# SymbioticLab/Oobleck

Measured on AMD Instinct MI355X. Metric: tokens/sec (whole node) GPT-2 1F1B, higher is better.
Workload: dtype bf16; 1 GPU; gpt2.yaml GPT-2-small 1F1B, global microbatch 128x1024 tokens, bf16; model=gpt2, global_batch=128, seq_len=1024, parallelism=pp1dp1

## Files before the change

include/oobleck_stage.h:

```cpp
#ifndef OOBLECK_STAGE_H
#define OOBLECK_STAGE_H

#include <stdint.h>

#ifdef __cplusplus
extern "C" {
#endif

enum {
  OB_KIND_EMBED = 0,
  OB_KIND_BLOCK = 1,
  OB_KIND_FINAL = 2
};

typedef struct ob_layer* ob_layer_t;

typedef struct {
  int32_t kind;
  int32_t n_embd;
  int32_t n_head;
  int32_t n_positions;
  int32_t vocab_size;
  int32_t max_batch;
  int32_t seq_len;
  int32_t n_slots;
  int32_t dtype;
} ob_layer_desc;

int64_t ob_layer_param_count(const ob_layer_desc* desc);

int ob_layer_create(const ob_layer_desc* desc, ob_layer_t* out);

enum {
  OB_DROP_EMBD = 0,
  OB_DROP_ATTN = 1,
  OB_DROP_RESID_ATTN = 2,
  OB_DROP_RESID_MLP = 3
};

typedef struct {
  float embd_pdrop;
  float resid_pdrop;
  float attn_pdrop;
  int32_t layer_id;
  uint64_t seed;
} ob_dropout_desc;

int ob_layer_create_ex(const ob_layer_desc* desc, const ob_dropout_desc* drop,
                       ob_layer_t* out);

int ob_layer_uses_flash(ob_layer_t l);

int ob_layer_set_training(ob_layer_t l, int on);

int ob_layer_set_dropout_tick(ob_layer_t l, uint64_t tick);

int ob_layer_bind(ob_layer_t l, void* params, void* grads);

int ob_layer_set_batch(ob_layer_t l, int32_t batch);

int ob_layer_forward(ob_layer_t l, int32_t slot, const void* in, void* out,
                     const int64_t* labels, void* stream);

int ob_layer_backward(ob_layer_t l, int32_t slot, const void* dout, void* din,
                      void* stream);

int ob_layer_destroy(ob_layer_t l);

int ob_layer_refresh_weights(ob_layer_t l, void* stream);

int ob_adamw_step(void* p, const void* g, void* m, void* v, int64_t n,
                  int32_t step, float lr, float beta1, float beta2, float eps,
                  float weight_decay, void* stream);


int64_t ob_sqnorm_ws_count(const int64_t* counts, int32_t n);

int ob_sqnorm_multi_f32(const void* const* ptrs, const int64_t* counts,
                        const int32_t* out_index, int32_t n, void* ws,
                        void* out, void* stream);

int ob_clip_finish(const void* sq, int32_t n, float max_norm, void* stats,
                   void* stream);

int ob_adamw_step_scaled(void* p, const void* g, void* m, void* v, int64_t n,
                         int32_t step, float lr, float beta1, float beta2,
                         float eps, float weight_decay, const void* clip_stats,
                         void* stream);


int ob_gemm_f32(int transA, int transB, int64_t M, int64_t N, int64_t K,
                float alpha, const void* A, int64_t lda,
                int64_t strideA1, int64_t strideA2,
                const void* B, int64_t ldb,
                int64_t strideB1, int64_t strideB2,
                float beta, void* C, int64_t ldc,
                int64_t strideC1, int64_t strideC2,
                int64_t n1, int64_t n2,
                const void* bias, const void* residual, int atomic, int splitk,
                void* stream);

int ob_layernorm_fwd_f32(const void* x, const void* w, const void* b, void* y,
                         void* mean, void* rstd, int64_t rows, int64_t H,
                         float eps, void* stream);
int ob_layernorm_bwd_f32(const void* x, const void* w, const void* mean,
                         const void* rstd, const void* dy, void* dx,
                         void* dw, void* db, int64_t rows, int64_t H,
                         int dx_accum, void* stream);

int ob_softmax_causal_fwd_f32(void* scores, int64_t batch, int64_t S,
                              float scale, void* stream);
int ob_softmax_causal_bwd_f32(const void* P, void* dP, int64_t batch,
                              int64_t S, void* stream);

int ob_gelu_fwd_f32(const void* u, void* g, int64_t n, void* stream);
int ob_gelu_bwd_f32(const void* u, const void* dg, void* du, int64_t n,
                    void* stream);

int ob_colsum_f32(const void* X, void* db, int64_t M, int64_t N, void* stream);

int ob_dropout_mask(uint64_t seed, int32_t layer_id, int32_t site,
                    uint64_t tick, float p, int64_t n, void* keep_u8,
                    void* stream);
int ob_dropout_scale_f32(uint64_t seed, int32_t layer_id, int32_t site,
                         uint64_t tick, float p, const void* x, void* y,
                         int64_t n, void* stream);
int ob_dropout_scale_bf16(uint64_t seed, int32_t layer_id, int32_t site,
                          uint64_t tick, float p, const void* x, void* y,
                          int64_t n, void* stream);
int ob_dropout_add_f32(uint64_t seed, int32_t layer_id, int32_t site,
                       uint64_t tick, float p, const void* t, const void* res,
                       void* y, int64_t n, void* stream);
int ob_dropout_add_bf16(uint64_t seed, int32_t layer_id, int32_t site,
                        uint64_t tick, float p, const void* t,
                        const void* res, void* y, int64_t n, void* stream);
int ob_dropout_scale_colsum_f32(uint64_t seed, int32_t layer_id, int32_t site,
                                uint64_t tick, float p, const void* dy,
                                void* dm, void* db, int64_t M, int64_t N,
                                void* stream);
int ob_dropout_scale_colsum_bf16(uint64_t seed, int32_t layer_id, int32_t site,
                                 uint64_t tick, float p, const void* dy,
                                 void* dm, void* db, int64_t M, int64_t N,
                                 void* stream);

int ob_gemm_bf16(int transA, int transB, int64_t M, int64_t N, int64_t K,
                 float alpha, const void* A, int64_t lda,
                 int64_t strideA1, int64_t strideA2,
                 const void* B, int64_t ldb,
                 int64_t strideB1, int64_t strideB2,
                 float beta, void* C, int64_t ldc,
                 int64_t strideC1, int64_t strideC2,
                 int64_t n1, int64_t n2,
                 const void* bias, const void* residual, int out_kind,
                 int splitk, void* stream);
int ob_gemm_bf16_route(int transA, int transB, int64_t M, int64_t N, int64_t K,
                       int64_t n1, int64_t n2, int out_kind, int splitk,
                       float beta, int aligned16, int env_mask,
                       const char* force, int32_t* out);

int ob_flash_fwd_nt_bf16(const void* qkv, void* O, void* lse, int64_t B,
                         int64_t Sq, int64_t H, int64_t nh, float scale,
                         void* stream);
int ob_flash_bwd_nt_bf16(const void* qkv, const void* dO, const void* lse,
                         const void* D, void* dqkv, void* dbias_qkv,
                         int64_t B, int64_t Sq, int64_t H, int64_t nh,
                         float scale, void* stream);
int ob_flash_bwd_nt_d_bf16(const void* qkv, const void* O, const void* dO,
                           const void* lse, void* D_ws, void* dqkv,
                           void* dbias_qkv, int64_t B, int64_t Sq, int64_t H,
                           int64_t nh, float scale, void* stream);
int ob_flash_fwd_nt_drop_bf16(const void* qkv, void* O, void* lse, int64_t B,
                              int64_t Sq, int64_t H, int64_t nh, float scale,
                              uint64_t seed, int32_t layer_id, uint64_t tick,
                              float p, void* stream);
int ob_flash_bwd_nt_d_drop_bf16(const void* qkv, const void* O, const void* dO,
                                const void* lse, void* D_ws, void* dqkv,
                                void* dbias_qkv, int64_t B, int64_t Sq,
                                int64_t H, int64_t nh, float scale,
                                uint64_t seed, int32_t layer_id, uint64_t tick,
                                float p, void* stream);
int ob_flash_fold_rows(int64_t kind, int64_t Sq, int64_t block, int64_t unit,
                       int64_t* row0, int64_t* first_tile, int64_t* n_tiles);
int64_t ob_flash_fold_grid(int64_t kind, int64_t Sq, int64_t Z);
int ob_flash_fold_id(int64_t kind, int64_t Sq, int64_t Z, int64_t id,
                     int64_t* z, int64_t* block);

int ob_f32_to_bf16(const void* x, void* y, int64_t n, void* stream);
int ob_f32_to_bf16_t(const void* x, void* y, int64_t rows, int64_t cols,
                     void* stream);
int ob_bf16_to_f32(const void* x, void* y, int64_t n, void* stream);

void ob_profile_enable(int on);
void ob_profile_reset(void);
int ob_profile_read(int fam, double* total_ms, long long* count);

const char* ob_last_error(void);

const char* ob_build_arch(void);

#ifdef __cplusplus
}
#endif
#endif
```

oobleck_amd/_ext.py:

```python
from __future__ import annotations

import ctypes
import pathlib

_LIB = None
SO_PATH = pathlib.Path(__file__).resolve().parent / "libob_stage.so"


class ObLayerDesc(ctypes.Structure):
    _fields_ = [
        ("kind", ctypes.c_int32),
        ("n_embd", ctypes.c_int32),
        ("n_head", ctypes.c_int32),
        ("n_positions", ctypes.c_int32),
        ("vocab_size", ctypes.c_int32),
        ("max_batch", ctypes.c_int32),
        ("seq_len", ctypes.c_int32),
        ("n_slots", ctypes.c_int32),
        ("dtype", ctypes.c_int32),
    ]


class ObDropoutDesc(ctypes.Structure):
    _fields_ = [
        ("embd_pdrop", ctypes.c_float),
        ("resid_pdrop", ctypes.c_float),
        ("attn_pdrop", ctypes.c_float),
        ("layer_id", ctypes.c_int32),
        ("seed", ctypes.c_uint64),
    ]


DROP_EMBD, DROP_ATTN, DROP_RESID_ATTN, DROP_RESID_MLP = 0, 1, 2, 3


def _configure(lib: ctypes.CDLL) -> ctypes.CDLL:
    i64, i32, f32, vp = ctypes.c_int64, ctypes.c_int32, ctypes.c_float, ctypes.c_void_p
    lib.ob_last_error.restype = ctypes.c_char_p
    lib.ob_build_arch.restype = ctypes.c_char_p
    lib.ob_layer_param_count.restype = i64
    lib.ob_layer_param_count.argtypes = [ctypes.POINTER(ObLayerDesc)]
    lib.ob_layer_create.argtypes = [ctypes.POINTER(ObLayerDesc),
                                    ctypes.POINTER(vp)]
    u64 = ctypes.c_uint64
    lib.ob_layer_create_ex.argtypes = [ctypes.POINTER(ObLayerDesc),
                                       ctypes.POINTER(ObDropoutDesc),
                                       ctypes.POINTER(vp)]
    lib.ob_layer_set_training.argtypes = [vp, i32]
    lib.ob_layer_uses_flash.argtypes = [vp]
    lib.ob_layer_set_dropout_tick.argtypes = [vp, u64]
    key = [u64, i32, i32, u64, f32]
    lib.ob_dropout_mask.argtypes = key + [i64, vp, vp]
    lib.ob_dropout_scale_f32.argtypes = key + [vp, vp, i64, vp]
    lib.ob_dropout_scale_bf16.argtypes = key + [vp, vp, i64, vp]
    lib.ob_dropout_add_f32.argtypes = key + [vp, vp, vp, i64, vp]
    lib.ob_dropout_add_bf16.argtypes = key + [vp, vp, vp, i64, vp]
    lib.ob_dropout_scale_colsum_f32.argtypes = key + [vp, vp, vp, i64, i64, vp]
    lib.ob_dropout_scale_colsum_bf16.argtypes = key + [vp, vp, vp, i64, i64,
                                                       vp]
    lib.ob_layer_bind.argtypes = [vp, vp, vp]
    lib.ob_layer_set_batch.argtypes = [vp, i32]
    lib.ob_layer_forward.argtypes = [vp, i32, vp, vp, vp, vp]
    lib.ob_layer_backward.argtypes = [vp, i32, vp, vp, vp]
    lib.ob_layer_destroy.argtypes = [vp]
    lib.ob_layer_refresh_weights.argtypes = [vp, vp]
    lib.ob_adamw_step.argtypes = [vp, vp, vp, vp, i64, i32, f32, f32, f32,
                                  f32, f32, vp]
    lib.ob_sqnorm_ws_count.restype = i64
    lib.ob_sqnorm_ws_count.argtypes = [ctypes.POINTER(i64), i32]
    lib.ob_sqnorm_multi_f32.argtypes = [ctypes.POINTER(vp),
                                        ctypes.POINTER(i64),
                                        ctypes.POINTER(i32), i32, vp, vp, vp]
    lib.ob_clip_finish.argtypes = [vp, i32, f32, vp, vp]
    lib.ob_adamw_step_scaled.argtypes = [vp, vp, vp, vp, i64, i32, f32, f32,
                                         f32, f32, f32, vp, vp]
    lib.ob_gemm_f32.argtypes = [i32, i32, i64, i64, i64, f32, vp, i64, i64,
                                i64, vp, i64, i64, i64, f32, vp, i64, i64,
                                i64, i64, i64, vp, vp, i32, i32, vp]
    lib.ob_layernorm_fwd_f32.argtypes = [vp, vp, vp, vp, vp, vp, i64, i64,
                                         f32, vp]
    lib.ob_layernorm_bwd_f32.argtypes = [vp, vp, vp, vp, vp, vp, vp, vp, i64,
                                         i64, i32, vp]
    lib.ob_softmax_causal_fwd_f32.argtypes = [vp, i64, i64, f32, vp]
    lib.ob_softmax_causal_bwd_f32.argtypes = [vp, vp, i64, i64, vp]
    lib.ob_gelu_fwd_f32.argtypes = [vp, vp, i64, vp]
    lib.ob_gelu_bwd_f32.argtypes = [vp, vp, vp, i64, vp]
    lib.ob_colsum_f32.argtypes = [vp, vp, i64, i64, vp]
    lib.ob_gemm_bf16.argtypes = [i32, i32, i64, i64, i64, f32, vp, i64, i64,
                                 i64, vp, i64, i64, i64, f32, vp, i64, i64,
                                 i64, i64, i64, vp, vp, i32, i32, vp]
    lib.ob_f32_to_bf16.argtypes = [vp, vp, i64, vp]
    lib.ob_f32_to_bf16_t.argtypes = [vp, vp, i64, i64, vp]
    lib.ob_f32_to_bf16_t_ld.argtypes = [vp, vp, i64, i64, i64, vp]
    lib.ob_bf16_to_f32.argtypes = [vp, vp, i64, vp]
    lib.ob_gelu_fwd_bf16.argtypes = [vp, vp, i64, vp]
    lib.ob_gelu_bwd_bf16.argtypes = [vp, vp, vp, i64, vp]
    lib.ob_ce_fwd_bf16.argtypes = [vp, vp, vp, vp, i64, i64, i64, i64, vp]
    lib.ob_ce_bwd_bf16.argtypes = [vp, vp, vp, vp, i64, i64, i64, i64, vp]
    lib.ob_embed_fwd_bf16.argtypes = [vp, vp, vp, vp, i64, i64, i64, vp]
    lib.ob_embed_bwd_bf16.argtypes = [vp, vp, vp, vp, i64, i64, i64, vp]
    lib.ob_softmax_causal_fwd_bf16.argtypes = [vp, i64, i64, f32, vp]
    lib.ob_softmax_causal_bwd_bf16.argtypes = [vp, vp, i64, i64, vp]
    lib.ob_transpose_bf16.argtypes = [vp, vp, i64, i64, vp]
    lib.ob_gemm_lt_bias.argtypes = [i32, i32, i64, i64, i64, f32, vp, i64,
                                    vp, i64, f32, vp, i64, i32, vp, vp]
    lib.ob_gemm_lt_f32.argtypes = [i32, i32, i64, i64, i64, f32, vp, i64,
                                   vp, i64, f32, vp, i64, vp]
    lib.ob_flash_fwd_bf16.argtypes = [vp, vp, vp, vp, i64, i64, i64, i64,
                                      f32, vp]
    lib.ob_transpose_bf16_b.argtypes = [vp, vp, i64, i64, i64, i64, i64,
                                        i64, i64, vp]
    lib.ob_layernorm_fwd_bf16.argtypes = [vp, vp, vp, vp, vp, vp, i64, i64,
                                          f32, vp]
    lib.ob_layernorm_bwd_bf16.argtypes = [vp, vp, vp, vp, vp, vp, vp, vp,
                                          i64, i64, i32, vp]
    lib.ob_colsum_bf16.argtypes = [vp, vp, i64, i64, vp]
    lib.ob_layernorm_fwd_copy_bf16.argtypes = [vp, vp, vp, vp, vp, vp, vp,
                                               i64, i64, f32, vp]
    lib.ob_layernorm_bwd_res_bf16.argtypes = [vp, vp, vp, vp, vp, vp, vp, vp,
                                              vp, vp, vp, i64, i64, vp]
    lib.ob_gelu_bwd_colsum_bf16.argtypes = [vp, vp, vp, vp, i64, i64, vp]
    lib.ob_gemm_lt.argtypes = [i32, i32, i64, i64, i64, f32, vp, i64, vp,
                               i64, f32, vp, i64, i32, vp]
    lib.ob_gemm_bf16_nt_8ph.argtypes = [vp, vp, vp, vp, vp, i64, i64, i64,
                                        i64, i64, i64, i64, i64, i64, i64,
                                        i64, i64, i64, i64, f32, f32, i32,
                                        i32, vp, i64]
    lib.ob_gemm_bf16_route.argtypes = [i32, i32, i64, i64, i64, i64, i64, i32,
                                       i32, f32, i32, i32, ctypes.c_char_p,
                                       ctypes.POINTER(ctypes.c_int32)]
    lib.ob_profile_enable.argtypes = [i32]
    lib.ob_profile_enable.restype = None
    lib.ob_profile_reset.argtypes = []
    lib.ob_profile_reset.restype = None
    lib.ob_profile_read.argtypes = [i32, ctypes.POINTER(ctypes.c_double),
                                    ctypes.POINTER(ctypes.c_longlong)]
    lib.ob_flash_dsum_bf16.argtypes = [vp, vp, vp, i64, i64, i64, i64, vp]
    lib.ob_flash_bwd_bf16.argtypes = [vp, vp, vp, vp, vp, vp, vp, vp, i64,
                                      i64, i64, i64, f32, vp]
    lib.ob_flash_fwd_nt_bf16.argtypes = [vp, vp, vp, i64, i64, i64, i64,
                                         f32, vp]
    lib.ob_flash_bwd_nt_bf16.argtypes = [vp, vp, vp, vp, vp, vp, i64, i64,
                                         i64, i64, f32, vp]
    lib.ob_flash_bwd_nt_d_bf16.argtypes = [vp, vp, vp, vp, vp, vp, vp, i64,
                                           i64, i64, i64, f32, vp]
    lib.ob_flash_fwd_nt_drop_bf16.argtypes = [vp, vp, vp, i64, i64, i64, i64,
                                              f32, u64, i32, u64, f32, vp]
    lib.ob_flash_bwd_nt_d_drop_bf16.argtypes = [vp, vp, vp, vp, vp, vp, vp,
                                                i64, i64, i64, i64, f32, u64,
                                                i32, u64, f32, vp]
    p64 = ctypes.POINTER(ctypes.c_int64)
    lib.ob_flash_fold_rows.argtypes = [i64, i64, i64, i64, p64, p64, p64]
    lib.ob_flash_fold_grid.argtypes = [i64, i64, i64]
    lib.ob_flash_fold_grid.restype = ctypes.c_int64
    lib.ob_flash_fold_id.argtypes = [i64, i64, i64, i64, p64, p64]
    return lib


def get_ext(build_if_missing: bool = True) -> ctypes.CDLL:
    global _LIB
    if _LIB is not None:
        return _LIB
    if not SO_PATH.exists():
        if build_if_missing:
            from .build import build
            try:
                build()
            except Exception as e:
                raise RuntimeError(
                    f"oobleck_amd: HIP extension missing and build failed: {e}. "
                    "The hot path has no fallback — run __graft_entry__.build().") from e
        else:
            raise RuntimeError(
                "oobleck_amd: HIP extension libob_stage.so is missing. "
                "The hot path has no fallback — run __graft_entry__.build().")
    _LIB = _configure(ctypes.CDLL(str(SO_PATH)))
    return _LIB


def check(rc: int, what: str = "") -> None:
    if rc != 0:
        err = get_ext().ob_last_error().decode()
        raise RuntimeError(f"oobleck_amd extension error in {what}: {err}")
```

oobleck_amd/csrc/ob_blaslt.hip:

```cpp
#include "ob_internal.h"

#include <hipblaslt/hipblaslt.h>

#include <cstdlib>
#include <map>
#include <tuple>

namespace {

struct LtPlan {
  hipblasLtMatmulDesc_t desc = nullptr;
  hipblasLtMatrixLayout_t la = nullptr, lb = nullptr, lc = nullptr;
  hipblasLtMatmulAlgo_t algo{};
  bool ok = false;
};

constexpr size_t kLtWs = 64u << 20;
using Key = std::tuple<int, int, int64_t, int64_t, int64_t, int64_t, int,
                       int, int, int>;

struct LtCtx {
  hipblasLtHandle_t h = nullptr;
  void* ws = nullptr;
  std::map<Key, LtPlan> plans;
};
std::map<void*, LtCtx> g_lt_by_stream;

LtCtx* lt_ctx(void* stream) {
  auto it = g_lt_by_stream.find(stream);
  if (it != g_lt_by_stream.end()) return &it->second;
  LtCtx ctx;
  if (hipblasLtCreate(&ctx.h) != HIPBLAS_STATUS_SUCCESS) return nullptr;
  if (hipMalloc(&ctx.ws, kLtWs) != hipSuccess) return nullptr;
  return &g_lt_by_stream.emplace(stream, ctx).first->second;
}

}

static int lt_matmul(int tA, int tB, int64_t M, int64_t N, int64_t K,
                     float alpha, const void* A, int64_t lda, const void* B,
                     int64_t ldb, float beta, void* C, int64_t ldc,
                     int c_f32, const void* bias, int ab_f32, void* stream,
                     const void* Cin = nullptr) {
  if (!Cin) Cin = C;
  LtCtx* ctx = lt_ctx(stream);
  if (!ctx) return ob_fail("hipblasLt per-stream context init failed");
  const Key key{tA,     tB,           M,
                N,      K,            ldc,
                c_f32,  beta != 0.f,  bias != nullptr,
                ab_f32};
  auto it = ctx->plans.find(key);
  if (it == ctx->plans.end()) {
    LtPlan p;
    const hipblasOperation_t opA = tB ? HIPBLAS_OP_T : HIPBLAS_OP_N;
    const hipblasOperation_t opB = tA ? HIPBLAS_OP_T : HIPBLAS_OP_N;
    const int64_t a_rows = tB ? K : N, a_cols = tB ? N : K;
    const int64_t b_rows = tA ? M : K, b_cols = tA ? K : M;
    hipblasLtMatmulDescCreate(&p.desc, HIPBLAS_COMPUTE_32F, HIP_R_32F);
    hipblasLtMatmulDescSetAttribute(p.desc, HIPBLASLT_MATMUL_DESC_TRANSA,
                                    &opA, sizeof(opA));
    hipblasLtMatmulDescSetAttribute(p.desc, HIPBLASLT_MATMUL_DESC_TRANSB,
                                    &opB, sizeof(opB));
    if (bias) {
      const hipblasLtEpilogue_t ep = HIPBLASLT_EPILOGUE_BIAS;
      hipblasLtMatmulDescSetAttribute(p.desc, HIPBLASLT_MATMUL_DESC_EPILOGUE,
                                      &ep, sizeof(ep));
      const int32_t bt = HIP_R_32F;
      hipblasLtMatmulDescSetAttribute(
          p.desc, HIPBLASLT_MATMUL_DESC_BIAS_DATA_TYPE, &bt, sizeof(bt));
      hipblasLtMatmulDescSetAttribute(
          p.desc, HIPBLASLT_MATMUL_DESC_BIAS_POINTER, &bias, sizeof(bias));
    }
    const hipDataType abt = ab_f32 ? HIP_R_32F : HIP_R_16BF;
    hipblasLtMatrixLayoutCreate(&p.la, abt, a_rows, a_cols, ldb);
    hipblasLtMatrixLayoutCreate(&p.lb, abt, b_rows, b_cols, lda);
    hipblasLtMatrixLayoutCreate(&p.lc, c_f32 ? HIP_R_32F : HIP_R_16BF, N, M,
                                ldc);
    hipblasLtMatmulPreference_t pref;
    hipblasLtMatmulPreferenceCreate(&pref);
    const uint64_t ws = kLtWs;
    hipblasLtMatmulPreferenceSetAttribute(
        pref, HIPBLASLT_MATMUL_PREF_MAX_WORKSPACE_BYTES, &ws, sizeof(ws));
    hipblasLtMatmulHeuristicResult_t res[1];
    int nres = 0;
    hipblasLtMatmulAlgoGetHeuristic(ctx->h, p.desc, p.la, p.lb, p.lc, p.lc,
                                    pref, 1, res, &nres);
    hipblasLtMatmulPreferenceDestroy(pref);
    if (nres > 0 && res[0].state == HIPBLAS_STATUS_SUCCESS) {
      p.algo = res[0].algo;
      p.ok = true;
    }
    it = ctx->plans.emplace(key, p).first;
  }
  const LtPlan& p = it->second;
  if (!p.ok) return -1;
  if (bias)
    hipblasLtMatmulDescSetAttribute(
        p.desc, HIPBLASLT_MATMUL_DESC_BIAS_POINTER, &bias, sizeof(bias));
  const hipblasStatus_t st = hipblasLtMatmul(
      ctx->h, p.desc, &alpha, B, p.la, A, p.lb, &beta, Cin, p.lc, C, p.lc,
      &p.algo, ctx->ws, kLtWs, reinterpret_cast<hipStream_t>(stream));
  if (st != HIPBLAS_STATUS_SUCCESS)
    return ob_fail("hipblasLtMatmul failed (%d)", (int)st);
  return 0;
}

extern "C" int ob_gemm_lt(int tA, int tB, int64_t M, int64_t N, int64_t K,
                          float alpha, const void* A, int64_t lda,
                          const void* B, int64_t ldb, float beta, void* C,
                          int64_t ldc, int c_f32, void* stream) {
  return lt_matmul(tA, tB, M, N, K, alpha, A, lda, B, ldb, beta, C, ldc,
                   c_f32, nullptr, 0, stream);
}

extern "C" int ob_gemm_lt_bias(int tA, int tB, int64_t M, int64_t N,
                               int64_t K, float alpha, const void* A,
                               int64_t lda, const void* B, int64_t ldb,
                               float beta, void* C, int64_t ldc, int c_f32,
                               const void* bias, void* stream) {
  return lt_matmul(tA, tB, M, N, K, alpha, A, lda, B, ldb, beta, C, ldc,
                   c_f32, bias, 0, stream);
}

extern "C" int ob_gemm_lt_bias_res(int tA, int tB, int64_t M, int64_t N,
                                   int64_t K, float alpha, const void* A,
                                   int64_t lda, const void* B, int64_t ldb,
                                   void* C, int64_t ldc, int c_f32,
                                   const void* bias, const void* residual,
                                   void* stream) {
  return lt_matmul(tA, tB, M, N, K, alpha, A, lda, B, ldb, 1.f, C, ldc,
                   c_f32, bias, 0, stream, residual);
}

extern "C" int ob_gemm_lt_f32(int tA, int tB, int64_t M, int64_t N,
                              int64_t K, float alpha, const void* A,
                              int64_t lda, const void* B, int64_t ldb,
                              float beta, void* C, int64_t ldc,
                              void* stream) {
  return lt_matmul(tA, tB, M, N, K, alpha, A, lda, B, ldb, beta, C, ldc, 1,
                   nullptr, 1, stream);
}
```

oobleck_amd/csrc/ob_internal.h:

```cpp
#pragma once
#include <hip/hip_runtime.h>

#include <cstdarg>
#include <cstdint>
#include <cstdio>
#include <cstdlib>

#include "../../include/oobleck_stage.h"

int ob_fail(const char* fmt, ...);

#define OB_HIP(x)                                                     \
  do {                                                                \
    hipError_t e_ = (x);                                              \
    if (e_ != hipSuccess)                                             \
      return ob_fail("%s:%d: %s", __FILE__, __LINE__,                 \
                     hipGetErrorString(e_));                          \
  } while (0)

#define OB_LAUNCH_CHECK()                                             \
  do {                                                                \
    hipError_t e_ = hipGetLastError();                                \
    if (e_ != hipSuccess)                                             \
      return ob_fail("%s:%d: launch: %s", __FILE__, __LINE__,         \
                     hipGetErrorString(e_));                          \
  } while (0)

inline bool ob_env_flag(const char* name, bool dflt) {
  const char* e = getenv(name);
  return (e && e[0] == (dflt ? '0' : '1')) ? !dflt : dflt;
}
inline int ob_env_int(const char* name, int dflt) {
  const char* e = getenv(name);
  return e ? atoi(e) : dflt;
}

enum {
  OB_PF_FC_FWD = 0,
  OB_PF_GEMM_FWD = 1,
  OB_PF_GEMM_DX = 2,
  OB_PF_GEMM_DW = 3,
  OB_PF_FLASH_FWD = 4,
  OB_PF_FLASH_BWD = 5,
  OB_PF_ATTN_MAT = 6,
  OB_PF_LN = 7,
  OB_PF_CE = 8,
  OB_PF_ELEM = 9,
  OB_PF_ADAMW = 10,
  OB_PF_NFAM = 11
};
bool ob_prof_on();
int ob_prof_beg(int fam, hipStream_t s);
void ob_prof_end(int fam, int slot, hipStream_t s);

#define OB_PROF(fid, strm, call)                                        \
  ({                                                                    \
    int _r;                                                             \
    if (ob_prof_on()) {                                                 \
      hipStream_t _ps = reinterpret_cast<hipStream_t>(strm);            \
      const int _fi = (fid);                                            \
      const int _slot = ob_prof_beg(_fi, _ps);                          \
      _r = (call);                                                      \
      ob_prof_end(_fi, _slot, _ps);                                     \
    } else {                                                            \
      _r = (call);                                                      \
    }                                                                   \
    _r;                                                                 \
  })

__device__ __forceinline__ void ob_adamw_update(
    float* __restrict__ p, float* __restrict__ m, float* __restrict__ v,
    int64_t i, float gi, float wd_factor, float step_size, float inv_sqrt_bc2,
    float beta1, float beta2, float eps) {
  float mi = beta1 * m[i] + (1.f - beta1) * gi;
  float vi = beta2 * v[i] + (1.f - beta2) * gi * gi;
  m[i] = mi;
  v[i] = vi;
  const float denom = sqrtf(vi) * inv_sqrt_bc2 + eps;
  p[i] = p[i] * wd_factor - step_size * mi / denom;
}

int ob_embed_fwd_f32(const int64_t* ids, const float* wte, const float* wpe,
                     float* out, int64_t B, int64_t S, int64_t H, void* stream);
int ob_embed_bwd_f32(const int64_t* ids, const float* dout, float* dwte,
                     float* dwpe, int64_t B, int64_t S, int64_t H, void* stream);
int ob_ce_fwd_f32(const float* logits, const int64_t* labels, float* lse,
                  float* loss, int64_t B, int64_t S, int64_t V, void* stream);
int ob_ce_bwd_f32(float* logits_to_dlogits, const int64_t* labels,
                  const float* lse, const float* dloss_or_null, int64_t B,
                  int64_t S, int64_t V, void* stream);

struct ob_drop_key;
int ob_drop_scale(const ob_drop_key& key, int bf16, const void* x, void* y,
                  int64_t n, void* stream);
int ob_drop_add(const ob_drop_key& key, int bf16, const void* t,
                const void* res, void* y, int64_t n, void* stream);
int ob_drop_scale_colsum(const ob_drop_key& key, int bf16, const void* dy,
                         void* dm, void* db, int64_t M, int64_t N,
                         void* stream);
int ob_embed_fwd_drop(const ob_drop_key& key, int bf16, const int64_t* ids,
                      const float* wte, const float* wpe, void* out, int64_t B,
                      int64_t Sq, int64_t H, void* stream);
int ob_embed_bwd_drop(const ob_drop_key& key, int bf16, const int64_t* ids,
                      const void* dout, float* dwte, float* dwpe, int64_t B,
                      int64_t Sq, int64_t H, void* stream);

extern "C" {
int ob_f32_to_bf16_t_ld(const void* x, void* y, int64_t rows, int64_t cols,
                        int64_t out_ld, void* stream);
int ob_layernorm_fwd_bf16(const void* x, const void* w, const void* b,
                          void* y, void* mean, void* rstd, int64_t rows,
                          int64_t H, float eps, void* stream);
int ob_layernorm_bwd_bf16(const void* x, const void* w, const void* mean,
                          const void* rstd, const void* dy, void* dx,
                          void* dw, void* db, int64_t rows, int64_t H,
                          int dx_accum, void* stream);
int ob_layernorm_fwd_copy_bf16(const void* x, const void* w, const void* b,
                               void* y, void* xcopy, void* mean, void* rstd,
                               int64_t rows, int64_t H, float eps,
                               void* stream);
int ob_layernorm_bwd_res_bf16(const void* x, const void* w, const void* mean,
                              const void* rstd, const void* dy,
                              const void* res, void* dx, void* dw, void* db,
                              void* sum_res, void* sum_dx, int64_t rows,
                              int64_t H, void* stream);
int ob_gelu_bwd_colsum_bf16(const void* u, const void* dg, void* du,
                            void* db, int64_t M, int64_t N, void* stream);
int ob_softmax_causal_fwd_bf16(void* scores, int64_t batch, int64_t Sq,
                               float scale, void* stream);
int ob_softmax_causal_bwd_bf16(const void* P, void* dP, int64_t batch,
                               int64_t Sq, void* stream);
int ob_gelu_fwd_bf16(const void* u, void* g, int64_t n, void* stream);
int ob_gelu_bwd_bf16(const void* u, const void* dg, void* du, int64_t n,
                     void* stream);
int ob_colsum_bf16(const void* X, void* db, int64_t M, int64_t N,
                   void* stream);
int ob_embed_fwd_bf16(const void* ids, const void* wte, const void* wpe,
                      void* out, int64_t B, int64_t Sq, int64_t H,
                      void* stream);
int ob_embed_bwd_bf16(const void* ids, const void* dout, void* dwte,
                      void* dwpe, int64_t B, int64_t Sq, int64_t H,
                      void* stream);
int ob_ce_fwd_bf16(const void* logits, const void* labels, void* lse,
                   void* loss, int64_t B, int64_t Sq, int64_t V, int64_t ld,
                   void* stream);
int ob_ce_bwd_bf16(void* logits, const void* labels, const void* lse,
                   const void* dloss, int64_t B, int64_t Sq, int64_t V,
                   int64_t ld, void* stream);
int ob_transpose_bf16(const void* in, void* out, int64_t R, int64_t C,
                      void* stream);
int ob_flash_fwd_bf16(const void* qkv, const void* VT, void* O, void* lse,
                      int64_t B, int64_t Sq, int64_t H, int64_t nh,
                      float scale, void* stream);
int ob_transpose_bf16_b(const void* in, void* out, int64_t R, int64_t C,
                        int64_t sIn1, int64_t sIn2, int64_t ldin, int64_t n1,
                        int64_t n2, void* stream);
int ob_flash_dsum_bf16(const void* O, const void* dO, void* D, int64_t B,
                       int64_t Sq, int64_t H, int64_t nh, void* stream);
int ob_flash_bwd_bf16(const void* qkv, const void* QT, const void* KT,
                      const void* dOT, const void* dO, const void* lse,
                      const void* D, void* dqkv, int64_t B, int64_t Sq,
                      int64_t H, int64_t nh, float scale, void* stream);
int ob_flash_fwd_nt_bf16(const void* qkv, void* O, void* lse, int64_t B,
                         int64_t Sq, int64_t H, int64_t nh, float scale,
                         void* stream);
int ob_flash_bwd_nt_bf16(const void* qkv, const void* dO, const void* lse,
                         const void* D, void* dqkv, void* dbias_qkv,
                         int64_t B, int64_t Sq, int64_t H, int64_t nh,
                         float scale, void* stream);
int ob_flash_bwd_nt_d_bf16(const void* qkv, const void* O, const void* dO,
                           const void* lse, void* D_ws, void* dqkv,
                           void* dbias_qkv, int64_t B, int64_t Sq, int64_t H,
                           int64_t nh, float scale, void* stream);
}
extern "C" int ob_gemm_lt(int tA, int tB, int64_t M, int64_t N, int64_t K,
                          float alpha, const void* A, int64_t lda,
                          const void* B, int64_t ldb, float beta, void* C,
                          int64_t ldc, int c_f32, void* stream);
extern "C" int ob_gemm_lt_bias(int tA, int tB, int64_t M, int64_t N,
                               int64_t K, float alpha, const void* A,
                               int64_t lda, const void* B, int64_t ldb,
                               float beta, void* C, int64_t ldc, int c_f32,
                               const void* bias, void* stream);
extern "C" int ob_gemm_lt_bias_res(int tA, int tB, int64_t M, int64_t N,
                                   int64_t K, float alpha, const void* A,
                                   int64_t lda, const void* B, int64_t ldb,
                                   void* C, int64_t ldc, int c_f32,
                                   const void* bias, const void* residual,
                                   void* stream);
extern "C" int ob_gemm_lt_f32(int tA, int tB, int64_t M, int64_t N,
                              int64_t K, float alpha, const void* A,
                              int64_t lda, const void* B, int64_t ldb,
                              float beta, void* C, int64_t ldc,
                              void* stream);
struct ob_bf16_gemm {
  const void* A = nullptr;
  const void* B = nullptr;
  void* C = nullptr;
  const void* bias = nullptr;
  const void* residual = nullptr;
  int64_t M = 0, N = 0, K = 0;
  int64_t lda = 0, ldb = 0, ldc = 0;
  int64_t sA1 = 0, sA2 = 0, sB1 = 0, sB2 = 0, sC1 = 0, sC2 = 0;
  int64_t n1 = 1, n2 = 1;
  float alpha = 1.f, beta = 0.f;
  int transA = 0, transB = 1;
  int out_kind = 0;
  int splitk = 1;
  int64_t Mr = 0;
  void* stream = nullptr;
};
int ob_gemm_bf16_run(const ob_bf16_gemm& g);
int ob_gemm_bf16_nt_dispatch(const ob_bf16_gemm& g);
int ob_gemm_bf16_nt256_dispatch(const ob_bf16_gemm& g, int BN);
int ob_gemm_bf16_nt_8ph_dispatch(const ob_bf16_gemm& g);
```

oobleck_amd/csrc/ob_layer.hip:

```cpp
#include "ob_internal.h"
#include "ob_philox.h"

#include <cmath>
#include <cstring>
#include <vector>

static inline hipStream_t S(void* s) { return reinterpret_cast<hipStream_t>(s); }
static inline int64_t i64min(int64_t a, int64_t b) { return a < b ? a : b; }
static inline int64_t i64max(int64_t a, int64_t b) { return a > b ? a : b; }


struct Workspace {
  float* dp = nullptr;
  float* bsh1 = nullptr;
  float* bsh2 = nullptr;
  float* dqkv = nullptr;
  float* b4h = nullptr;
  float* t1 = nullptr;
  float* t2 = nullptr;
  float* s1 = nullptr;
  float* s2 = nullptr;
  float* pd_f = nullptr;
  float* pd_b = nullptr;
  float* dm1 = nullptr;
  float* dm2 = nullptr;
  int64_t sz_dp = 0, sz_bsh = 0, sz_bsh2 = 0, sz_dqkv = 0, sz_b4h = 0,
          sz_t1 = 0, sz_t2 = 0, sz_s1 = 0, sz_s2 = 0, sz_pd_f = 0,
          sz_pd_b = 0, sz_dm1 = 0, sz_dm2 = 0;
};
static Workspace g_ws;

struct SideSync {
  hipStream_t stream = nullptr;
  hipEvent_t ring[128] = {};
  int ri = 0;
  bool ready = false;
};
static SideSync g_side;

static hipEvent_t side_evt() {
  hipEvent_t e = g_side.ring[g_side.ri & 127];
  g_side.ri++;
  return e;
}

static int side_init() {
  if (g_side.ready) return 0;
  OB_HIP(hipStreamCreateWithFlags(&g_side.stream, hipStreamNonBlocking));
  for (int i = 0; i < 128; i++)
    OB_HIP(hipEventCreateWithFlags(&g_side.ring[i], hipEventDisableTiming));
  g_side.ready = true;
  return 0;
}

#define OB_SIDE_FENCE(from, to)                      \
  do {                                               \
    hipEvent_t ev_ = side_evt();                     \
    OB_HIP(hipEventRecord(ev_, (from)));             \
    OB_HIP(hipStreamWaitEvent((to), ev_, 0));        \
  } while (0)


struct ProfFam {
  static constexpr int RING = 64;
  hipEvent_t beg[RING] = {}, end[RING] = {};
  bool pending[RING] = {};
  int head = 0;
  double total_ms = 0.0;
  long long count = 0;
};
static struct {
  bool on = false;
  ProfFam fam[OB_PF_NFAM];
} g_prof;

static void prof_drain_slot(ProfFam& f, int i) {
  if (!f.pending[i]) return;
  hipEventSynchronize(f.end[i]);
  float ms = 0.f;
  if (hipEventElapsedTime(&ms, f.beg[i], f.end[i]) == hipSuccess)
    f.total_ms += ms;
  f.pending[i] = false;
}

bool ob_prof_on() { return g_prof.on; }

int ob_prof_beg(int fam, hipStream_t s) {
  ProfFam& f = g_prof.fam[fam];
  const int i = f.head;
  if (!f.beg[i]) {
    hipEventCreate(&f.beg[i]);
    hipEventCreate(&f.end[i]);
  }
  prof_drain_slot(f, i);
  hipEventRecord(f.beg[i], s);
  return i;
}

void ob_prof_end(int fam, int slot, hipStream_t s) {
  ProfFam& f = g_prof.fam[fam];
  hipEventRecord(f.end[slot], s);
  f.pending[slot] = true;
  f.count++;
  f.head = (slot + 1) % ProfFam::RING;
}

extern "C" void ob_profile_enable(int on) { g_prof.on = on != 0; }

extern "C" void ob_profile_reset(void) {
  for (auto& f : g_prof.fam) {
    for (int i = 0; i < ProfFam::RING; i++)
      if (f.pending[i]) {
        hipEventSynchronize(f.end[i]);
        f.pending[i] = false;
      }
    f.total_ms = 0.0;
    f.count = 0;
    f.head = 0;
  }
}

extern "C" int ob_profile_read(int fam, double* total_ms, long long* count) {
  if (fam < 0 || fam >= OB_PF_NFAM) return ob_fail("profile_read: bad fam");
  ProfFam& f = g_prof.fam[fam];
  for (int i = 0; i < ProfFam::RING; i++) prof_drain_slot(f, i);
  *total_ms = f.total_ms;
  *count = f.count;
  return 0;
}

static int ws_ensure(float** buf, int64_t* cur, int64_t need) {
  if (need <= *cur) return 0;
  if (*buf) OB_HIP(hipFree(*buf));
  *buf = nullptr;
  *cur = 0;
  OB_HIP(hipMalloc(buf, need * sizeof(float)));
  *cur = need;
  return 0;
}


struct ob_layer {
  ob_layer_desc d;
  int B;
  float* params = nullptr;
  float* grads = nullptr;
  float* stash = nullptr;
  int64_t slot_stride = 0;
  int64_t* ids = nullptr;
  int64_t o_x = 0, o_mean1 = 0, o_rstd1 = 0, o_ln1 = 0, o_qkv = 0, o_p = 0,
          o_attnm = 0, o_hmid = 0, o_mean2 = 0, o_rstd2 = 0, o_ln2 = 0,
          o_u = 0, o_g = 0, o_logits = 0, o_lse = 0;
  __bf16* shadows = nullptr;
  int64_t v_pad = 0;
  int64_t sh_qkv = 0, sh_qkv_t = 0, sh_ap = 0, sh_ap_t = 0, sh_fc = 0,
          sh_fc_t = 0, sh_mp = 0, sh_mp_t = 0, sh_lm = 0, sh_lm_t = 0;
  int64_t shadow_count = 0;
  bool flash = false;
  float p_embd = 0.f, p_resid = 0.f, p_attn = 0.f;
  int32_t layer_id = 0;
  uint64_t seed = 0;
  bool training = true;
  uint64_t next_tick = 0;
  std::vector<uint8_t> slot_drop;
  std::vector<uint64_t> slot_tick;
};

static bool has_dropout(const ob_layer* l) {
  return l->p_embd > 0.f || l->p_resid > 0.f || l->p_attn > 0.f;
}
static ob_drop_key drop_key(const ob_layer* l, int slot, int site, float p) {
  return ob_drop_make_key(l->seed, l->layer_id, site, l->slot_tick[slot], p);
}

static bool flash_tr() {
  static const bool on = ob_env_flag("OB_FLASH_TR", true);
  return on;
}

static bool flash_drop() {
  static const bool on = ob_env_flag("OB_FLASH_DROP", true);
  return on;
}

static bool flash_eligible(const ob_layer_desc* d, float attn_pdrop = 0.f) {
  if (attn_pdrop > 0.f && !(flash_tr() && flash_drop())) return false;
  static const bool on = ob_env_flag("OB_BF16_FLASH", true);
  return on && d->dtype == 1 && d->n_embd / d->n_head == 64 &&
         d->seq_len % 128 == 0;
}

struct BlockParams {
  int64_t ln1_w, ln1_b, w_qkv, b_qkv, w_attnproj, b_attnproj, ln2_w, ln2_b,
      w_fc, b_fc, w_mlpproj, b_mlpproj, total;
};
static BlockParams block_params(int64_t H) {
  BlockParams p;
  int64_t o = 0;
  p.ln1_w = o; o += H;
  p.ln1_b = o; o += H;
  p.w_qkv = o; o += H * 3 * H;
  p.b_qkv = o; o += 3 * H;
  p.w_attnproj = o; o += H * H;
  p.b_attnproj = o; o += H;
  p.ln2_w = o; o += H;
  p.ln2_b = o; o += H;
  p.w_fc = o; o += H * 4 * H;
  p.b_fc = o; o += 4 * H;
  p.w_mlpproj = o; o += 4 * H * H;
  p.b_mlpproj = o; o += H;
  p.total = o;
  return p;
}

extern "C" int64_t ob_layer_param_count(const ob_layer_desc* d) {
  const int64_t H = d->n_embd, V = d->vocab_size, P = d->n_positions;
  switch (d->kind) {
    case OB_KIND_EMBED: return V * H + P * H;
    case OB_KIND_BLOCK: return block_params(H).total;
    case OB_KIND_FINAL: return 2 * H + V * H;
  }
  return -1;
}

static int layer_create(const ob_layer_desc* d, const ob_dropout_desc* drop,
                        ob_layer_t* out) {
  if (!d || !out) return ob_fail("create: null arg");
  if (d->kind < 0 || d->kind > 2) return ob_fail("create: bad kind");
  if (d->seq_len > 2048)
    return ob_fail("create: seq_len > 2048 unsupported in round 1");
  if (d->n_slots < 1) return ob_fail("create: n_slots < 1");
  if (drop) {
    if (!ob_drop_p_ok(drop->embd_pdrop) || !ob_drop_p_ok(drop->resid_pdrop) ||
        !ob_drop_p_ok(drop->attn_pdrop))
      return ob_fail("create_ex: dropout probabilities must be in [0,1)");
    if (drop->layer_id < 0 || drop->layer_id >= (1 << 24))
      return ob_fail("create_ex: layer_id out of range");
  }
  ob_layer* l = new ob_layer();
  l->d = *d;
  l->B = d->max_batch;
  l->slot_drop.assign(d->n_slots, 0);
  l->slot_tick.assign(d->n_slots, 0);
  if (drop) {
    if (d->kind == OB_KIND_EMBED) l->p_embd = drop->embd_pdrop;
    if (d->kind == OB_KIND_BLOCK) {
      l->p_resid = drop->resid_pdrop;
      l->p_attn = drop->attn_pdrop;
    }
    l->layer_id = drop->layer_id;
    l->seed = drop->seed;
  }
  const int64_t Bm = d->max_batch, Sq = d->seq_len, H = d->n_embd,
                nh = d->n_head, V = d->vocab_size;
  const int64_t BS = Bm * Sq, BSH = BS * H;
  int64_t o = 0;
  switch (d->kind) {
    case OB_KIND_EMBED:
      l->slot_stride = 0;
      break;
    case OB_KIND_BLOCK:
      l->o_x = o; o += BSH;
      l->o_mean1 = o; o += BS;
      l->o_rstd1 = o; o += BS;
      l->o_ln1 = o; o += BSH;
      l->o_qkv = o; o += BS * 3 * H;
      l->flash = flash_eligible(d, l->p_attn);
      l->o_p = o; o += l->flash ? Bm * nh * Sq : Bm * nh * Sq * Sq;
      l->o_attnm = o; o += BSH;
      l->o_hmid = o; o += BSH;
      l->o_mean2 = o; o += BS;
      l->o_rstd2 = o; o += BS;
      l->o_ln2 = o; o += BSH;
      l->o_u = o; o += BS * 4 * H;
      l->o_g = o; o += BS * 4 * H;
      l->slot_stride = o;
      break;
    case OB_KIND_FINAL:
      l->o_x = o; o += BSH;
      l->o_mean1 = o; o += BS;
      l->o_rstd1 = o; o += BS;
      l->o_ln1 = o; o += BSH;
      l->o_logits = o; o += BS * V;
      l->o_lse = o; o += BS;
      l->slot_stride = o;
      break;
  }
  if (l->slot_stride > 0) {
    if (hipMalloc(&l->stash, (size_t)l->slot_stride * d->n_slots *
                                 sizeof(float)) != hipSuccess) {
      delete l;
      return ob_fail("create: stash hipMalloc of %lld floats failed",
                     (long long)(l->slot_stride * d->n_slots));
    }
  }
  if (d->kind == OB_KIND_EMBED || d->kind == OB_KIND_FINAL) {
    if (hipMalloc(&l->ids, (size_t)BS * d->n_slots * sizeof(int64_t)) !=
        hipSuccess) {
      if (l->stash) hipFree(l->stash);
      delete l;
      return ob_fail("create: ids hipMalloc failed");
    }
  }
  l->v_pad = (V + 255) / 256 * 256;
  if (d->dtype == 1) {
    int64_t o2 = 0;
    if (d->kind == OB_KIND_BLOCK) {
      l->sh_qkv = o2; o2 += 3 * H * H;
      l->sh_qkv_t = o2; o2 += 3 * H * H;
      l->sh_ap = o2; o2 += H * H;
      l->sh_ap_t = o2; o2 += H * H;
      l->sh_fc = o2; o2 += 4 * H * H;
      l->sh_fc_t = o2; o2 += 4 * H * H;
      l->sh_mp = o2; o2 += 4 * H * H;
      l->sh_mp_t = o2; o2 += 4 * H * H;
    } else if (d->kind == OB_KIND_FINAL) {
      l->sh_lm = o2; o2 += l->v_pad * H;
      l->sh_lm_t = o2; o2 += H * l->v_pad;
    }
    l->shadow_count = o2;
    if (o2 > 0) {
      if (hipMalloc(&l->shadows, (size_t)o2 * sizeof(__bf16)) != hipSuccess)
        return ob_fail("create: shadow hipMalloc failed");
      OB_HIP(hipMemset(l->shadows, 0, (size_t)o2 * sizeof(__bf16)));
    }
  }
  if (d->kind == OB_KIND_BLOCK) {
    if (!l->flash &&
        ws_ensure(&g_ws.dp, &g_ws.sz_dp, Bm * nh * Sq * Sq))
      return 1;
    if (ws_ensure(&g_ws.dqkv, &g_ws.sz_dqkv, BS * 3 * H)) return 1;
    if (ws_ensure(&g_ws.b4h, &g_ws.sz_b4h, BS * 4 * H)) return 1;
    if (d->dtype == 1) {
      if (l->flash && flash_tr()) {
        if (ws_ensure(&g_ws.t1, &g_ws.sz_t1, Bm * nh * Sq)) return 1;
      } else {
        if (ws_ensure(&g_ws.t1, &g_ws.sz_t1, (4 * H * BS + 1) / 2)) return 1;
        if (ws_ensure(&g_ws.t2, &g_ws.sz_t2, (4 * H * BS + 1) / 2)) return 1;
      }
      if (ws_ensure(&g_ws.s1, &g_ws.sz_s1, (4 * H * BS + 1) / 2)) return 1;
      if (ws_ensure(&g_ws.s2, &g_ws.sz_s2, (4 * H * BS + 1) / 2)) return 1;
      if (side_init()) return 1;
    }
  }
  if (d->kind == OB_KIND_FINAL && d->dtype == 1) {
    if (ws_ensure(&g_ws.t1, &g_ws.sz_t1, (l->v_pad * BS + 1) / 2)) return 1;
    if (ws_ensure(&g_ws.t2, &g_ws.sz_t2, (4 * H * BS + 1) / 2)) return 1;
    if (ws_ensure(&g_ws.s1, &g_ws.sz_s1, (l->v_pad * BS + 1) / 2)) return 1;
    if (ws_ensure(&g_ws.s2, &g_ws.sz_s2, (4 * H * BS + 1) / 2)) return 1;
    if (side_init()) return 1;
  }
  if (d->kind != OB_KIND_EMBED) {
    const int64_t need = BSH;
    if (ws_ensure(&g_ws.bsh1, &g_ws.sz_bsh, need)) return 1;
    if (ws_ensure(&g_ws.bsh2, &g_ws.sz_bsh2, need)) return 1;
  }
  if (l->p_attn > 0.f && !l->flash) {
    if (ws_ensure(&g_ws.pd_f, &g_ws.sz_pd_f, Bm * nh * Sq * Sq)) return 1;
    if (ws_ensure(&g_ws.pd_b, &g_ws.sz_pd_b, Bm * nh * Sq * Sq)) return 1;
  }
  if (l->p_resid > 0.f) {
    if (ws_ensure(&g_ws.dm1, &g_ws.sz_dm1, BSH)) return 1;
    if (ws_ensure(&g_ws.dm2, &g_ws.sz_dm2, BSH)) return 1;
  }
  *out = l;
  return 0;
}

extern "C" int ob_layer_create(const ob_layer_desc* d, ob_layer_t* out) {
  return layer_create(d, nullptr, out);
}

extern "C" int ob_layer_create_ex(const ob_layer_desc* d,
                                  const ob_dropout_desc* drop,
                                  ob_layer_t* out) {
  return layer_create(d, drop, out);
}

extern "C" int ob_layer_uses_flash(ob_layer_t l) {
  return l && l->flash ? 1 : 0;
}

extern "C" int ob_layer_set_training(ob_layer_t l, int on) {
  if (!l) return ob_fail("set_training: null layer");
  l->training = on != 0;
  return 0;
}

extern "C" int ob_layer_set_dropout_tick(ob_layer_t l, uint64_t tick) {
  if (!l) return ob_fail("set_dropout_tick: null layer");
  l->next_tick = tick;
  return 0;
}

extern "C" int ob_layer_bind(ob_layer_t l, void* params, void* grads) {
  if (!l) return ob_fail("bind: null layer");
  l->params = (float*)params;
  l->grads = (float*)grads;
  return 0;
}

extern "C" int ob_layer_set_batch(ob_layer_t l, int32_t batch) {
  if (!l) return ob_fail("set_batch: null layer");
  if (batch < 1 || batch > l->d.max_batch)
    return ob_fail("set_batch: %d out of range (max %d)", batch,
                   l->d.max_batch);
  l->B = batch;
  return 0;
}

extern "C" int ob_layer_destroy(ob_layer_t l) {
  if (!l) return 0;
  if (l->stash) hipFree(l->stash);
  if (l->ids) hipFree(l->ids);
  if (l->shadows) hipFree(l->shadows);
  delete l;
  return 0;
}

extern "C" int ob_layer_refresh_weights(ob_layer_t l, void* stream) {
  if (!l) return ob_fail("refresh: null layer");
  if (l->d.dtype != 1) return 0;
  if (!l->params) return ob_fail("refresh: params not bound");
  const int64_t H = l->d.n_embd, V = l->d.vocab_size;
  const float* p = l->params;
  __bf16* sh = l->shadows;
  switch (l->d.kind) {
    case OB_KIND_EMBED:
      return 0;
    case OB_KIND_BLOCK: {
      const BlockParams bp = block_params(H);
      if (ob_f32_to_bf16(p + bp.w_qkv, sh + l->sh_qkv, 3 * H * H, stream) ||
          ob_f32_to_bf16_t_ld(p + bp.w_qkv, sh + l->sh_qkv_t, H, 3 * H, H,
                              stream) ||
          ob_f32_to_bf16(p + bp.w_attnproj, sh + l->sh_ap, H * H, stream) ||
          ob_f32_to_bf16_t_ld(p + bp.w_attnproj, sh + l->sh_ap_t, H, H, H,
                              stream) ||
          ob_f32_to_bf16(p + bp.w_fc, sh + l->sh_fc, 4 * H * H, stream) ||
          ob_f32_to_bf16_t_ld(p + bp.w_fc, sh + l->sh_fc_t, H, 4 * H, H,
                              stream) ||
          ob_f32_to_bf16(p + bp.w_mlpproj, sh + l->sh_mp, 4 * H * H, stream) ||
          ob_f32_to_bf16_t_ld(p + bp.w_mlpproj, sh + l->sh_mp_t, 4 * H, H,
                              4 * H, stream))
        return 1;
      return 0;
    }
    case OB_KIND_FINAL:
      if (ob_f32_to_bf16(p + 2 * H, sh + l->sh_lm, V * H, stream) ||
          ob_f32_to_bf16_t_ld(p + 2 * H, sh + l->sh_lm_t, V, H, l->v_pad,
                              stream))
        return 1;
      return 0;
  }
  return ob_fail("refresh: bad kind");
}

static int gemm(int tA, int tB, int64_t M, int64_t N, int64_t K, float alpha,
                const float* A, int64_t lda, int64_t sA1, int64_t sA2,
                const float* B, int64_t ldb, int64_t sB1, int64_t sB2,
                float beta, float* C, int64_t ldc, int64_t sC1, int64_t sC2,
                int64_t n1, int64_t n2, const float* bias, const float* R,
                int atomic, int splitk, void* stream) {
  static const bool no_lt = ob_env_flag("OB_NO_BLASLT", false);
  if (!no_lt && !bias && !R && !atomic && splitk <= 1 && n1 == 1 &&
      n2 == 1 && M * N >= 512 * 512) {
    const int r = ob_gemm_lt_f32(tA, tB, M, N, K, alpha, A, lda, B, ldb,
                                 beta, C, ldc, stream);
    if (r >= 0) return r;
  }
  return ob_gemm_f32(tA, tB, M, N, K, alpha, A, lda, sA1, sA2, B, ldb, sB1,
                     sB2, beta, C, ldc, sC1, sC2, n1, n2, bias, R, atomic,
                     splitk, stream);
}

static int pick_splitk(int64_t M, int64_t N, int64_t K) {
  const int64_t tiles = ((M + 127) / 128) * ((N + 127) / 128);
  int sk = 1;
  while (sk < 16 && tiles * sk < 512 && (K / (sk * 2)) >= 256) sk *= 2;
  return sk;
}

static int gemm_dx_splitk(int tB, int64_t M, int64_t N, int64_t K,
                          float alpha, const float* A, int64_t lda,
                          const float* B, int64_t ldb, float* C, int64_t ldc,
                          void* stream) {
  static const bool no_lt = ob_env_flag("OB_NO_BLASLT", false);
  if (!no_lt) {
    const int r = ob_gemm_lt_f32(0, tB, M, N, K, alpha, A, lda, B, ldb, 0.f,
                                 C, ldc, stream);
    if (r >= 0) return r;
  }
  const int64_t tiles = ((M + 127) / 128) * ((N + 127) / 128);
  int sk = 1;
  while (sk < 16 && tiles * sk < 1024 && (K / (sk * 2)) >= 512) sk *= 2;
  if (sk == 1)
    return ob_gemm_f32(0, tB, M, N, K, alpha, A, lda, 0, 0, B, ldb, 0, 0,
                       0.f, C, ldc, 0, 0, 1, 1, nullptr, nullptr, 0, 1,
                       stream);
  OB_HIP(hipMemsetAsync(C, 0, (size_t)M * ldc * sizeof(float), S(stream)));
  return ob_gemm_f32(0, tB, M, N, K, alpha, A, lda, 0, 0, B, ldb, 0, 0, 0.f,
                     C, ldc, 0, 0, 1, 1, nullptr, nullptr, 1, sk, stream);
}


static int block_forward(ob_layer* l, int slot, const float* in, float* out,
                         void* stream) {
  const int64_t Sq = l->d.seq_len, H = l->d.n_embd, nh = l->d.n_head;
  const int64_t B = l->B, BS = B * Sq;
  const int64_t hd = H / nh;
  float* st = l->stash + (int64_t)slot * l->slot_stride;
  const float* p = l->params;
  const BlockParams bp = block_params(H);
  const bool dA = l->slot_drop[slot] && l->p_attn > 0.f;
  const bool dR = l->slot_drop[slot] && l->p_resid > 0.f;

  float* x = st + l->o_x;
  OB_HIP(hipMemcpyAsync(x, in, BS * H * sizeof(float), hipMemcpyDeviceToDevice,
                        S(stream)));
  float* ln1 = st + l->o_ln1;
  if (ob_layernorm_fwd_f32(x, p + bp.ln1_w, p + bp.ln1_b, ln1,
                           st + l->o_mean1, st + l->o_rstd1, BS, H, 1e-5f,
                           stream))
    return 1;
  float* qkv = st + l->o_qkv;
  if (gemm(0, 0, BS, 3 * H, H, 1.f, ln1, H, 0, 0, p + bp.w_qkv, 3 * H, 0, 0,
           0.f, qkv, 3 * H, 0, 0, 1, 1, p + bp.b_qkv, nullptr, 0, 1, stream))
    return 1;
  float* P = st + l->o_p;
  if (gemm(0, 1, Sq, Sq, hd, 1.f,
           qkv, 3 * H, Sq * 3 * H, hd,
           qkv + H, 3 * H, Sq * 3 * H, hd,
           0.f, P, Sq, nh * Sq * Sq, Sq * Sq, B, nh, nullptr, nullptr, 0, 1,
           stream))
    return 1;
  if (ob_softmax_causal_fwd_f32(P, B * nh, Sq, 1.f / sqrtf((float)hd), stream))
    return 1;
  const float* Pv = P;
  if (dA) {
    if (ob_drop_scale(drop_key(l, slot, OB_DROP_ATTN, l->p_attn), 0, P,
                      g_ws.pd_f, B * nh * Sq * Sq, stream))
      return 1;
    Pv = g_ws.pd_f;
  }
  float* am = st + l->o_attnm;
  if (gemm(0, 0, Sq, hd, Sq, 1.f, Pv, Sq, nh * Sq * Sq, Sq * Sq, qkv + 2 * H,
           3 * H, Sq * 3 * H, hd, 0.f, am, H, Sq * H, hd, B, nh, nullptr,
           nullptr, 0, 1, stream))
    return 1;
  float* hmid = st + l->o_hmid;
  if (gemm(0, 0, BS, H, H, 1.f, am, H, 0, 0, p + bp.w_attnproj, H, 0, 0, 0.f,
           hmid, H, 0, 0, 1, 1, p + bp.b_attnproj, dR ? nullptr : x, 0, 1,
           stream))
    return 1;
  if (dR && ob_drop_add(drop_key(l, slot, OB_DROP_RESID_ATTN, l->p_resid), 0,
                        hmid, x, hmid, BS * H, stream))
    return 1;
  float* ln2 = st + l->o_ln2;
  if (ob_layernorm_fwd_f32(hmid, p + bp.ln2_w, p + bp.ln2_b, ln2,
                           st + l->o_mean2, st + l->o_rstd2, BS, H, 1e-5f,
                           stream))
    return 1;
  float* u = st + l->o_u;
  if (gemm(0, 0, BS, 4 * H, H, 1.f, ln2, H, 0, 0, p + bp.w_fc, 4 * H, 0, 0,
           0.f, u, 4 * H, 0, 0, 1, 1, p + bp.b_fc, nullptr, 0, 1, stream))
    return 1;
  float* gact = st + l->o_g;
  if (ob_gelu_fwd_f32(u, gact, BS * 4 * H, stream)) return 1;
  if (gemm(0, 0, BS, H, 4 * H, 1.f, gact, 4 * H, 0, 0, p + bp.w_mlpproj, H, 0,
           0, 0.f, out, H, 0, 0, 1, 1, p + bp.b_mlpproj, dR ? nullptr : hmid,
           0, 1, stream))
    return 1;
  if (dR && ob_drop_add(drop_key(l, slot, OB_DROP_RESID_MLP, l->p_resid), 0,
                        out, hmid, out, BS * H, stream))
    return 1;
  return 0;
}

static int final_forward(ob_layer* l, int slot, const float* in, float* out,
                         const int64_t* labels, void* stream) {
  const int64_t Sq = l->d.seq_len, H = l->d.n_embd, V = l->d.vocab_size;
  const int64_t B = l->B, BS = B * Sq;
  float* st = l->stash + (int64_t)slot * l->slot_stride;
  const float* p = l->params;
  if (!labels) return ob_fail("final_forward: labels required");

  float* x = st + l->o_x;
  OB_HIP(hipMemcpyAsync(x, in, BS * H * sizeof(float), hipMemcpyDeviceToDevice,
                        S(stream)));
  int64_t* labs = l->ids + (int64_t)slot * (int64_t)l->d.max_batch * Sq;
  OB_HIP(hipMemcpyAsync(labs, labels, BS * sizeof(int64_t),
                        hipMemcpyDeviceToDevice, S(stream)));
  float* lnf = st + l->o_ln1;
  if (ob_layernorm_fwd_f32(x, p + 0, p + H, lnf, st + l->o_mean1,
                           st + l->o_rstd1, BS, H, 1e-5f, stream))
    return 1;
  float* logits = st + l->o_logits;
  if (gemm(0, 1, BS, V, H, 1.f, lnf, H, 0, 0, p + 2 * H, H, 0, 0, 0.f, logits,
           V, 0, 0, 1, 1, nullptr, nullptr, 0, 1, stream))
    return 1;
  OB_HIP(hipMemsetAsync(out, 0, sizeof(float), S(stream)));
  if (ob_ce_fwd_f32(logits, labs, st + l->o_lse, out, B, Sq, V, stream))
    return 1;
  return 0;
}


static int linear_bf(const void* in, int64_t M, int64_t K, const void* W,
                     int64_t N, const float* bias, const void* res, void* out,
                     void* stream) {
  ob_bf16_gemm g;
  g.A = in, g.B = W, g.C = out, g.bias = bias, g.residual = res;
  g.M = M, g.N = N, g.K = K, g.lda = K, g.ldb = K, g.ldc = N;
  g.stream = stream;
  return ob_gemm_bf16_run(g);
}

static ob_bf16_gemm attn_gemm(int tA, int tB, int64_t M, int64_t N, int64_t K,
                              float alpha, int64_t B, int64_t nh,
                              void* stream) {
  ob_bf16_gemm g;
  g.transA = tA, g.transB = tB, g.M = M, g.N = N, g.K = K, g.alpha = alpha;
  g.n1 = B, g.n2 = nh, g.stream = stream;
  return g;
}

static int dw_bf16_ws(const __bf16* act, int64_t actw, const __bf16* dY,
                      int64_t dyw, int64_t BS, float* gout, int64_t ldc,
                      float* w1, float* w2, void* stream) {
  static const bool no_lt = ob_env_flag("OB_NO_BLASLT", false);
  if (!no_lt && ldc == dyw) {
    const int r = ob_gemm_lt(1, 0, actw, dyw, BS, 1.f, act, actw, dY, dyw,
                             1.f, gout, ldc, 1, stream);
    if (r >= 0) return r;
  }
  ob_bf16_gemm g;
  g.C = gout, g.M = actw, g.N = dyw, g.K = BS, g.ldc = ldc;
  g.out_kind = 2, g.splitk = pick_splitk(actw, dyw, BS), g.stream = stream;
  if ((actw % 128) || (dyw % 128) || (BS % 128)) {
    g.transA = 1, g.transB = 0;
    g.A = act, g.lda = actw, g.B = dY, g.ldb = dyw;
    return ob_gemm_bf16_run(g);
  }
  __bf16* XT = (__bf16*)w1;
  __bf16* DYT = (__bf16*)w2;
  if (ob_transpose_bf16(act, XT, BS, actw, stream)) return 1;
  if (ob_transpose_bf16(dY, DYT, BS, dyw, stream)) return 1;
  g.A = XT, g.lda = BS, g.B = DYT, g.ldb = BS;
  return ob_gemm_bf16_run(g);
}

static int block_forward_bf16(ob_layer* l, int slot, const __bf16* in,
                              __bf16* out, void* stream) {
  const int64_t Sq = l->d.seq_len, H = l->d.n_embd, nh = l->d.n_head;
  const int64_t B = l->B, BS = B * Sq;
  const int64_t hd = H / nh;
  float* st = l->stash + (int64_t)slot * l->slot_stride;
  const float* p = l->params;
  const __bf16* sh = l->shadows;
  const BlockParams bp = block_params(H);
  const bool dA = l->slot_drop[slot] && l->p_attn > 0.f;
  const bool dR = l->slot_drop[slot] && l->p_resid > 0.f;

  __bf16* x = (__bf16*)(st + l->o_x);
  __bf16* ln1 = (__bf16*)(st + l->o_ln1);
  if (OB_PROF(OB_PF_LN, stream,
              ob_layernorm_fwd_copy_bf16(in, p + bp.ln1_w, p + bp.ln1_b, ln1,
                                         x, st + l->o_mean1, st + l->o_rstd1,
                                         BS, H, 1e-5f, stream)))
    return 1;
  __bf16* qkv = (__bf16*)(st + l->o_qkv);
  if (OB_PROF(OB_PF_GEMM_FWD, stream,
              linear_bf(ln1, BS, H, sh + l->sh_qkv_t, 3 * H, p + bp.b_qkv,
                        nullptr, qkv, stream)))
    return 1;
  __bf16* am = (__bf16*)(st + l->o_attnm);
  if (l->flash && flash_tr()) {
    float* lseP = st + l->o_p;
    if (dA) {
      if (OB_PROF(OB_PF_FLASH_FWD, stream,
                  ob_flash_fwd_nt_drop_bf16(qkv, am, lseP, B, Sq, H, nh,
                                            1.f / sqrtf((float)hd), l->seed,
                                            l->layer_id, l->slot_tick[slot],
                                            l->p_attn, stream)))
        return 1;
    } else if (OB_PROF(OB_PF_FLASH_FWD, stream,
                       ob_flash_fwd_nt_bf16(qkv, am, lseP, B, Sq, H, nh,
                                            1.f / sqrtf((float)hd), stream)))
      return 1;
  } else if (l->flash) {
    __bf16* VTw = (__bf16*)g_ws.t2;
    if (OB_PROF(OB_PF_FLASH_FWD, stream,
                ob_transpose_bf16_b(qkv + 2 * H, VTw, Sq, 64, Sq * 3 * H, 64,
                                    3 * H, B, nh, stream)))
      return 1;
    float* lseP = st + l->o_p;
    if (OB_PROF(OB_PF_FLASH_FWD, stream,
                ob_flash_fwd_bf16(qkv, VTw, am, lseP, B, Sq, H, nh,
                                  1.f / sqrtf((float)hd), stream)))
      return 1;
  } else {
    __bf16* P = (__bf16*)(st + l->o_p);
    ob_bf16_gemm qk = attn_gemm(0, 1, Sq, Sq, hd, 1.f, B, nh, stream);
    qk.A = qkv, qk.lda = 3 * H, qk.sA1 = Sq * 3 * H, qk.sA2 = hd;
    qk.B = qkv + H, qk.ldb = 3 * H, qk.sB1 = Sq * 3 * H, qk.sB2 = hd;
    qk.C = P, qk.ldc = Sq, qk.sC1 = nh * Sq * Sq, qk.sC2 = Sq * Sq;
    if (OB_PROF(OB_PF_ATTN_MAT, stream, ob_gemm_bf16_run(qk))) return 1;
    if (OB_PROF(OB_PF_ATTN_MAT, stream,
                ob_softmax_causal_fwd_bf16(P, B * nh, Sq,
                                           1.f / sqrtf((float)hd), stream)))
      return 1;
    const __bf16* Pv = P;
    if (dA) {
      if (OB_PROF(OB_PF_ELEM, stream,
                  ob_drop_scale(drop_key(l, slot, OB_DROP_ATTN, l->p_attn), 1,
                                P, g_ws.pd_f, B * nh * Sq * Sq, stream)))
        return 1;
      Pv = (const __bf16*)g_ws.pd_f;
    }
    ob_bf16_gemm pv = attn_gemm(0, 0, Sq, hd, Sq, 1.f, B, nh, stream);
    pv.A = Pv, pv.lda = Sq, pv.sA1 = nh * Sq * Sq, pv.sA2 = Sq * Sq;
    pv.B = qkv + 2 * H, pv.ldb = 3 * H, pv.sB1 = Sq * 3 * H, pv.sB2 = hd;
    pv.C = am, pv.ldc = H, pv.sC1 = Sq * H, pv.sC2 = hd;
    if (OB_PROF(OB_PF_ATTN_MAT, stream, ob_gemm_bf16_run(pv))) return 1;
  }
  __bf16* hmid = (__bf16*)(st + l->o_hmid);
  if (OB_PROF(OB_PF_GEMM_FWD, stream,
              linear_bf(am, BS, H, sh + l->sh_ap_t, H, p + bp.b_attnproj,
                        dR ? nullptr : x, hmid, stream)))
    return 1;
  if (dR &&
      OB_PROF(OB_PF_ELEM, stream,
              ob_drop_add(drop_key(l, slot, OB_DROP_RESID_ATTN, l->p_resid), 1,
                          hmid, x, hmid, BS * H, stream)))
    return 1;
  __bf16* ln2 = (__bf16*)(st + l->o_ln2);
  if (OB_PROF(OB_PF_LN, stream,
              ob_layernorm_fwd_bf16(hmid, p + bp.ln2_w, p + bp.ln2_b, ln2,
                                    st + l->o_mean2, st + l->o_rstd2, BS, H,
                                    1e-5f, stream)))
    return 1;
  __bf16* u = (__bf16*)(st + l->o_u);
  if (OB_PROF(OB_PF_FC_FWD, stream,
              linear_bf(ln2, BS, H, sh + l->sh_fc_t, 4 * H, p + bp.b_fc,
                        nullptr, u, stream)))
    return 1;
  __bf16* gact = (__bf16*)(st + l->o_g);
  if (OB_PROF(OB_PF_ELEM, stream,
              ob_gelu_fwd_bf16(u, gact, BS * 4 * H, stream)))
    return 1;
  if (OB_PROF(OB_PF_GEMM_FWD, stream,
              linear_bf(gact, BS, 4 * H, sh + l->sh_mp_t, H,
                        p + bp.b_mlpproj, dR ? nullptr : hmid, out, stream)))
    return 1;
  if (dR &&
      OB_PROF(OB_PF_ELEM, stream,
              ob_drop_add(drop_key(l, slot, OB_DROP_RESID_MLP, l->p_resid), 1,
                          out, hmid, out, BS * H, stream)))
    return 1;
  return 0;
}

static int final_forward_bf16(ob_layer* l, int slot, const __bf16* in,
                              float* out, const int64_t* labels,
                              void* stream) {
  const int64_t Sq = l->d.seq_len, H = l->d.n_embd, V = l->d.vocab_size;
  const int64_t B = l->B, BS = B * Sq;
  float* st = l->stash + (int64_t)slot * l->slot_stride;
  const float* p = l->params;
  if (!labels) return ob_fail("final_forward_bf16: labels required");

  __bf16* x = (__bf16*)(st + l->o_x);
  int64_t* labs = l->ids + (int64_t)slot * (int64_t)l->d.max_batch * Sq;
  OB_HIP(hipMemcpyAsync(labs, labels, BS * sizeof(int64_t),
                        hipMemcpyDeviceToDevice, S(stream)));
  __bf16* lnf = (__bf16*)(st + l->o_ln1);
  if (OB_PROF(OB_PF_LN, stream,
              ob_layernorm_fwd_copy_bf16(in, p + 0, p + H, lnf, x,
                                         st + l->o_mean1, st + l->o_rstd1,
                                         BS, H, 1e-5f, stream)))
    return 1;
  __bf16* logits = (__bf16*)(st + l->o_logits);
  if (OB_PROF(OB_PF_GEMM_FWD, stream,
              linear_bf(lnf, BS, H, l->shadows + l->sh_lm, l->v_pad, nullptr,
                        nullptr, logits, stream)))
    return 1;
  OB_HIP(hipMemsetAsync(out, 0, sizeof(float), S(stream)));
  if (OB_PROF(OB_PF_CE, stream,
              ob_ce_fwd_bf16(logits, labs, st + l->o_lse, out, B, Sq, V,
                             l->v_pad, stream)))
    return 1;
  return 0;
}

static int block_backward_bf16(ob_layer* l, int slot, const __bf16* dout,
                               __bf16* din, void* stream) {
  const int64_t Sq = l->d.seq_len, H = l->d.n_embd, nh = l->d.n_head;
  const int64_t B = l->B, BS = B * Sq;
  const int64_t hd = H / nh;
  const float scale = 1.f / sqrtf((float)hd);
  float* st = l->stash + (int64_t)slot * l->slot_stride;
  const float* p = l->params;
  float* g = l->grads;
  const __bf16* sh = l->shadows;
  const BlockParams bp = block_params(H);

  __bf16* x = (__bf16*)(st + l->o_x);
  __bf16* ln1 = (__bf16*)(st + l->o_ln1);
  __bf16* qkv = (__bf16*)(st + l->o_qkv);
  __bf16* P = (__bf16*)(st + l->o_p);
  __bf16* am = (__bf16*)(st + l->o_attnm);
  __bf16* hmid = (__bf16*)(st + l->o_hmid);
  __bf16* ln2 = (__bf16*)(st + l->o_ln2);
  __bf16* u = (__bf16*)(st + l->o_u);
  __bf16* gact = (__bf16*)(st + l->o_g);

  __bf16* DY4 = (__bf16*)g_ws.b4h;
  __bf16* DLN = (__bf16*)g_ws.bsh1;
  __bf16* DATT = (__bf16*)g_ws.bsh2;
  __bf16* DQKV = (__bf16*)g_ws.dqkv;
  __bf16* DP = (__bf16*)g_ws.dp;
  const bool dA = l->slot_drop[slot] && l->p_attn > 0.f;
  const bool dR = l->slot_drop[slot] && l->p_resid > 0.f;

  void* const side = (void*)g_side.stream;
  OB_SIDE_FENCE(S(stream), g_side.stream);

  const __bf16* dmlp = dout;
  if (dR) {
    if (OB_PROF(OB_PF_ELEM, stream,
                ob_drop_scale_colsum(
                    drop_key(l, slot, OB_DROP_RESID_MLP, l->p_resid), 1, dout,
                    g_ws.dm2, g + bp.b_mlpproj, BS, H, stream)))
      return 1;
    dmlp = (const __bf16*)g_ws.dm2;
    OB_SIDE_FENCE(S(stream), g_side.stream);
  }
  if (OB_PROF(OB_PF_GEMM_DX, stream,
              linear_bf(dmlp, BS, H, sh + l->sh_mp, 4 * H, nullptr, nullptr,
                        DY4, stream)))
    return 1;
  if (OB_PROF(OB_PF_GEMM_DW, side,
              dw_bf16_ws(gact, 4 * H, dmlp, H, BS, g + bp.w_mlpproj, H,
                         g_ws.s1, g_ws.s2, side)))
    return 1;
  if (OB_PROF(OB_PF_ELEM, stream,
              ob_gelu_bwd_colsum_bf16(u, DY4, DY4, g + bp.b_fc, BS, 4 * H,
                                      stream)))
    return 1;
  OB_SIDE_FENCE(S(stream), g_side.stream);
  if (OB_PROF(OB_PF_GEMM_DW, side,
              dw_bf16_ws(ln2, H, DY4, 4 * H, BS, g + bp.w_fc, 4 * H, g_ws.s1,
                         g_ws.s2, side)))
    return 1;
  if (OB_PROF(OB_PF_GEMM_DX, stream,
              linear_bf(DY4, BS, 4 * H, sh + l->sh_fc, H, nullptr, nullptr,
                        DLN, stream)))
    return 1;
  if (OB_PROF(OB_PF_LN, stream,
              ob_layernorm_bwd_res_bf16(hmid, p + bp.ln2_w, st + l->o_mean2,
                                        st + l->o_rstd2, DLN, dout, din,
                                        g + bp.ln2_w, g + bp.ln2_b,
                                        dR ? nullptr : g + bp.b_mlpproj,
                                        dR ? nullptr : g + bp.b_attnproj,
                                        BS, H, stream)))
    return 1;
  const __bf16* dap = din;
  if (dR) {
    if (OB_PROF(OB_PF_ELEM, stream,
                ob_drop_scale_colsum(
                    drop_key(l, slot, OB_DROP_RESID_ATTN, l->p_resid), 1, din,
                    g_ws.dm1, g + bp.b_attnproj, BS, H, stream)))
      return 1;
    dap = (const __bf16*)g_ws.dm1;
  }
  OB_SIDE_FENCE(S(stream), g_side.stream);
  if (OB_PROF(OB_PF_GEMM_DX, stream,
              linear_bf(dap, BS, H, sh + l->sh_ap, H, nullptr, nullptr, DATT,
                        stream)))
    return 1;
  if (OB_PROF(OB_PF_GEMM_DW, side,
              dw_bf16_ws(am, H, dap, H, BS, g + bp.w_attnproj, H, g_ws.s1,
                         g_ws.s2, side)))
    return 1;
  hipEvent_t ev_din_done = side_evt();
  OB_HIP(hipEventRecord(ev_din_done, g_side.stream));
  const bool flash_nt = l->flash && flash_tr();
  if (flash_nt) {
    float* Dbuf = g_ws.t1;
    const float* lseP = st + l->o_p;
    if (dA) {
      if (OB_PROF(OB_PF_FLASH_BWD, stream,
                  ob_flash_bwd_nt_d_drop_bf16(qkv, am, DATT, lseP, Dbuf, DQKV,
                                              g + bp.b_qkv, B, Sq, H, nh,
                                              scale, l->seed, l->layer_id,
                                              l->slot_tick[slot], l->p_attn,
                                              stream)))
        return 1;
    } else if (OB_PROF(OB_PF_FLASH_BWD, stream,
                       ob_flash_bwd_nt_d_bf16(qkv, am, DATT, lseP, Dbuf, DQKV,
                                              g + bp.b_qkv, B, Sq, H, nh,
                                              scale, stream)))
      return 1;
  } else if (l->flash) {
    const int64_t BSH = BS * H;
    __bf16* QTw = (__bf16*)g_ws.t1;
    __bf16* KTw = QTw + BSH;
    __bf16* dOTw = KTw + BSH;
    float* Dbuf = g_ws.t1 + (3 * BSH + 1) / 2;
    const float* lseP = st + l->o_p;
    if (OB_PROF(OB_PF_FLASH_BWD, stream,
                ob_transpose_bf16_b(qkv, QTw, Sq, 64, Sq * 3 * H, 64, 3 * H,
                                    B, nh, stream)))
      return 1;
    if (OB_PROF(OB_PF_FLASH_BWD, stream,
                ob_transpose_bf16_b(qkv + H, KTw, Sq, 64, Sq * 3 * H, 64,
                                    3 * H, B, nh, stream)))
      return 1;
    if (OB_PROF(OB_PF_FLASH_BWD, stream,
                ob_transpose_bf16_b(DATT, dOTw, Sq, 64, Sq * H, 64, H, B, nh,
                                    stream)))
      return 1;
    if (OB_PROF(OB_PF_FLASH_BWD, stream,
                ob_flash_dsum_bf16(am, DATT, Dbuf, B, Sq, H, nh, stream)))
      return 1;
    if (OB_PROF(OB_PF_FLASH_BWD, stream,
                ob_flash_bwd_bf16(qkv, QTw, KTw, dOTw, DATT, lseP, Dbuf,
                                  DQKV, B, Sq, H, nh, scale, stream)))
      return 1;
  } else {
    ob_bf16_gemm dp = attn_gemm(0, 1, Sq, Sq, hd, 1.f, B, nh, stream);
    dp.A = DATT, dp.lda = H, dp.sA1 = Sq * H, dp.sA2 = hd;
    dp.B = qkv + 2 * H, dp.ldb = 3 * H, dp.sB1 = Sq * 3 * H, dp.sB2 = hd;
    dp.C = DP, dp.ldc = Sq, dp.sC1 = nh * Sq * Sq, dp.sC2 = Sq * Sq;
    if (OB_PROF(OB_PF_ATTN_MAT, stream, ob_gemm_bf16_run(dp))) return 1;
    const __bf16* Pv = P;
    if (dA) {
      const ob_drop_key ka = drop_key(l, slot, OB_DROP_ATTN, l->p_attn);
      if (OB_PROF(OB_PF_ELEM, stream,
                  ob_drop_scale(ka, 1, P, g_ws.pd_b, B * nh * Sq * Sq,
                                stream)))
        return 1;
      if (OB_PROF(OB_PF_ELEM, stream,
                  ob_drop_scale(ka, 1, DP, DP, B * nh * Sq * Sq, stream)))
        return 1;
      Pv = (const __bf16*)g_ws.pd_b;
    }
    if (OB_PROF(OB_PF_ATTN_MAT, stream,
                ob_softmax_causal_bwd_bf16(P, DP, B * nh, Sq, stream)))
      return 1;
    ob_bf16_gemm dq = attn_gemm(0, 0, Sq, hd, Sq, scale, B, nh, stream);
    dq.A = DP, dq.lda = Sq, dq.sA1 = nh * Sq * Sq, dq.sA2 = Sq * Sq;
    dq.B = qkv + H, dq.ldb = 3 * H, dq.sB1 = Sq * 3 * H, dq.sB2 = hd;
    dq.C = DQKV, dq.ldc = 3 * H, dq.sC1 = Sq * 3 * H, dq.sC2 = hd;
    if (OB_PROF(OB_PF_ATTN_MAT, stream, ob_gemm_bf16_run(dq))) return 1;
    ob_bf16_gemm dk = dq;
    dk.transA = 1, dk.B = qkv, dk.C = DQKV + H;
    if (OB_PROF(OB_PF_ATTN_MAT, stream, ob_gemm_bf16_run(dk))) return 1;
    ob_bf16_gemm dv = dk;
    dv.alpha = 1.f, dv.A = Pv, dv.C = DQKV + 2 * H;
    dv.B = DATT, dv.ldb = H, dv.sB1 = Sq * H, dv.sB2 = hd;
    if (OB_PROF(OB_PF_ATTN_MAT, stream, ob_gemm_bf16_run(dv))) return 1;
  }
  OB_SIDE_FENCE(S(stream), g_side.stream);
  if (!flash_nt &&
      OB_PROF(OB_PF_ELEM, side,
              ob_colsum_bf16(DQKV, g + bp.b_qkv, BS, 3 * H, side)))
    return 1;
  if (OB_PROF(OB_PF_GEMM_DW, side,
              dw_bf16_ws(ln1, H, DQKV, 3 * H, BS, g + bp.w_qkv, 3 * H,
                         g_ws.s1, g_ws.s2, side)))
    return 1;
  if (OB_PROF(OB_PF_GEMM_DX, stream,
              linear_bf(DQKV, BS, 3 * H, sh + l->sh_qkv, H, nullptr, nullptr,
                        DLN, stream)))
    return 1;
  OB_HIP(hipStreamWaitEvent(S(stream), ev_din_done, 0));
  if (OB_PROF(OB_PF_LN, stream,
              ob_layernorm_bwd_bf16(x, p + bp.ln1_w, st + l->o_mean1,
                                    st + l->o_rstd1, DLN, din, g + bp.ln1_w,
                                    g + bp.ln1_b, BS, H, 1, stream)))
    return 1;
  OB_SIDE_FENCE(g_side.stream, S(stream));
  return 0;
}

static int final_backward_bf16(ob_layer* l, int slot, const float* dout,
                               __bf16* din, void* stream) {
  const int64_t Sq = l->d.seq_len, H = l->d.n_embd, V = l->d.vocab_size;
  const int64_t B = l->B, BS = B * Sq;
  float* st = l->stash + (int64_t)slot * l->slot_stride;
  const float* p = l->params;
  float* g = l->grads;
  __bf16* x = (__bf16*)(st + l->o_x);
  __bf16* lnf = (__bf16*)(st + l->o_ln1);
  __bf16* logits = (__bf16*)(st + l->o_logits);
  int64_t* labs = l->ids + (int64_t)slot * (int64_t)l->d.max_batch * Sq;
  __bf16* DLN = (__bf16*)g_ws.bsh1;

  if (OB_PROF(OB_PF_CE, stream,
              ob_ce_bwd_bf16(logits, labs, st + l->o_lse, dout, B, Sq, V,
                             l->v_pad, stream)))
    return 1;
  {
    OB_SIDE_FENCE(S(stream), g_side.stream);
    void* const side = (void*)g_side.stream;
    static const bool no_lt = ob_env_flag("OB_NO_BLASLT", false);
    int r = -1;
    if (!no_lt)
      r = OB_PROF(OB_PF_GEMM_DW, side,
                  ob_gemm_lt(1, 0, V, H, BS, 1.f, logits, l->v_pad, lnf, H,
                             1.f, g + 2 * H, H, 1, side));
    if (r > 0) return 1;
    if (r < 0) {
      __bf16* DLT = (__bf16*)g_ws.s1;
      __bf16* LNT = (__bf16*)g_ws.s2;
      if (ob_transpose_bf16(logits, DLT, BS, l->v_pad, side)) return 1;
      if (ob_transpose_bf16(lnf, LNT, BS, H, side)) return 1;
      ob_bf16_gemm dw;
      dw.A = DLT, dw.lda = BS, dw.B = LNT, dw.ldb = BS;
      dw.C = g + 2 * H, dw.ldc = H, dw.M = l->v_pad, dw.N = H, dw.K = BS;
      dw.out_kind = 2, dw.splitk = 2, dw.Mr = V, dw.stream = side;
      if (OB_PROF(OB_PF_GEMM_DW, side, ob_gemm_bf16_nt_dispatch(dw)))
        return 1;
    }
  }
  if (OB_PROF(OB_PF_GEMM_DX, stream,
              linear_bf(logits, BS, l->v_pad, l->shadows + l->sh_lm_t, H,
                        nullptr, nullptr, DLN, stream)))
    return 1;
  if (OB_PROF(OB_PF_LN, stream,
              ob_layernorm_bwd_bf16(x, p + 0, st + l->o_mean1,
                                    st + l->o_rstd1, DLN, din, g + 0, g + H,
                                    BS, H, 0, stream)))
    return 1;
  OB_SIDE_FENCE(g_side.stream, S(stream));
  return 0;
}

extern "C" int ob_layer_forward(ob_layer_t l, int32_t slot, const void* in,
                                void* out, const int64_t* labels,
                                void* stream) {
  if (!l) return ob_fail("forward: null layer");
  if (!l->params) return ob_fail("forward: params not bound");
  if (slot < 0 || slot >= l->d.n_slots) return ob_fail("forward: bad slot");
  const bool drop = l->training && has_dropout(l);
  l->slot_drop[slot] = drop ? 1 : 0;
  l->slot_tick[slot] = l->next_tick;
  if (drop) l->next_tick++;
  switch (l->d.kind) {
    case OB_KIND_EMBED: {
      const int64_t Sq = l->d.seq_len, H = l->d.n_embd, V = l->d.vocab_size;
      const int64_t BS = (int64_t)l->B * Sq;
      int64_t* ids = l->ids + (int64_t)slot * (int64_t)l->d.max_batch * Sq;
      OB_HIP(hipMemcpyAsync(ids, in, BS * sizeof(int64_t),
                            hipMemcpyDeviceToDevice, S(stream)));
      if (drop)
        return OB_PROF(OB_PF_ELEM, stream,
                       ob_embed_fwd_drop(
                           drop_key(l, slot, OB_DROP_EMBD, l->p_embd),
                           l->d.dtype == 1, ids, l->params, l->params + V * H,
                           out, l->B, Sq, H, stream));
      if (l->d.dtype == 1)
        return OB_PROF(OB_PF_ELEM, stream,
                       ob_embed_fwd_bf16(ids, l->params, l->params + V * H,
                                         out, l->B, Sq, H, stream));
      return OB_PROF(OB_PF_ELEM, stream,
                     ob_embed_fwd_f32(ids, l->params, l->params + V * H,
                                      (float*)out, l->B, Sq, H, stream));
    }
    case OB_KIND_BLOCK:
      if (l->d.dtype == 1)
        return block_forward_bf16(l, slot, (const __bf16*)in, (__bf16*)out,
                                  stream);
      return block_forward(l, slot, (const float*)in, (float*)out, stream);
    case OB_KIND_FINAL:
      if (l->d.dtype == 1)
        return final_forward_bf16(l, slot, (const __bf16*)in, (float*)out,
                                  labels, stream);
      return final_forward(l, slot, (const float*)in, (float*)out, labels,
                           stream);
  }
  return ob_fail("forward: bad kind");
}


static int block_backward(ob_layer* l, int slot, const float* dout, float* din,
                          void* stream) {
  const int64_t Sq = l->d.seq_len, H = l->d.n_embd, nh = l->d.n_head;
  const int64_t B = l->B, BS = B * Sq;
  const int64_t hd = H / nh;
  const float scale = 1.f / sqrtf((float)hd);
  float* st = l->stash + (int64_t)slot * l->slot_stride;
  const float* p = l->params;
  float* g = l->grads;
  const BlockParams bp = block_params(H);

  float* x = st + l->o_x;
  float* ln1 = st + l->o_ln1;
  float* qkv = st + l->o_qkv;
  float* P = st + l->o_p;
  float* am = st + l->o_attnm;
  float* hmid = st + l->o_hmid;
  float* ln2 = st + l->o_ln2;
  float* u = st + l->o_u;
  float* gact = st + l->o_g;

  float* DY4 = g_ws.b4h;
  float* DLN = g_ws.bsh1;
  float* DATT = g_ws.bsh2;
  float* DQKV = g_ws.dqkv;
  float* DP = g_ws.dp;
  const bool dA = l->slot_drop[slot] && l->p_attn > 0.f;
  const bool dR = l->slot_drop[slot] && l->p_resid > 0.f;

  OB_HIP(hipMemcpyAsync(din, dout, BS * H * sizeof(float),
                        hipMemcpyDeviceToDevice, S(stream)));
  const float* dmlp = dout;
  if (dR) {
    if (ob_drop_scale_colsum(drop_key(l, slot, OB_DROP_RESID_MLP, l->p_resid),
                             0, dout, g_ws.dm2, g + bp.b_mlpproj, BS, H,
                             stream))
      return 1;
    dmlp = g_ws.dm2;
  }
  if (gemm(0, 1, BS, 4 * H, H, 1.f, dmlp, H, 0, 0, p + bp.w_mlpproj, H, 0, 0,
           0.f, DY4, 4 * H, 0, 0, 1, 1, nullptr, nullptr, 0, 1, stream))
    return 1;
  if (gemm(1, 0, 4 * H, H, BS, 1.f, gact, 4 * H, 0, 0, dmlp, H, 0, 0, 1.f,
           g + bp.w_mlpproj, H, 0, 0, 1, 1, nullptr, nullptr, 1,
           pick_splitk(4 * H, H, BS), stream))
    return 1;
  if (!dR && ob_colsum_f32(dout, g + bp.b_mlpproj, BS, H, stream)) return 1;
  if (ob_gelu_bwd_f32(u, DY4, DY4, BS * 4 * H, stream)) return 1;
  if (gemm(1, 0, H, 4 * H, BS, 1.f, ln2, H, 0, 0, DY4, 4 * H, 0, 0, 1.f,
           g + bp.w_fc, 4 * H, 0, 0, 1, 1, nullptr, nullptr, 1,
           pick_splitk(H, 4 * H, BS), stream))
    return 1;
  if (ob_colsum_f32(DY4, g + bp.b_fc, BS, 4 * H, stream)) return 1;
  if (gemm_dx_splitk(1, BS, H, 4 * H, 1.f, DY4, 4 * H, p + bp.w_fc, 4 * H,
                     DLN, H, stream))
    return 1;
  if (ob_layernorm_bwd_f32(hmid, p + bp.ln2_w, st + l->o_mean2,
                           st + l->o_rstd2, DLN, din, g + bp.ln2_w,
                           g + bp.ln2_b, BS, H, 1, stream))
    return 1;
  const float* dap = din;
  if (dR) {
    if (ob_drop_scale_colsum(drop_key(l, slot, OB_DROP_RESID_ATTN, l->p_resid),
                             0, din, g_ws.dm1, g + bp.b_attnproj, BS, H,
                             stream))
      return 1;
    dap = g_ws.dm1;
  }
  if (gemm_dx_splitk(1, BS, H, H, 1.f, dap, H, p + bp.w_attnproj, H, DATT,
                     H, stream))
    return 1;
  if (gemm(1, 0, H, H, BS, 1.f, am, H, 0, 0, dap, H, 0, 0, 1.f,
           g + bp.w_attnproj, H, 0, 0, 1, 1, nullptr, nullptr, 1,
           pick_splitk(H, H, BS), stream))
    return 1;
  if (!dR && ob_colsum_f32(din, g + bp.b_attnproj, BS, H, stream)) return 1;
  if (gemm(0, 1, Sq, Sq, hd, 1.f, DATT, H, Sq * H, hd, qkv + 2 * H, 3 * H,
           Sq * 3 * H, hd, 0.f, DP, Sq, nh * Sq * Sq, Sq * Sq, B, nh, nullptr,
           nullptr, 0, 1, stream))
    return 1;
  const float* Pv = P;
  if (dA) {
    const ob_drop_key ka = drop_key(l, slot, OB_DROP_ATTN, l->p_attn);
    if (ob_drop_scale(ka, 0, P, g_ws.pd_b, B * nh * Sq * Sq, stream)) return 1;
    if (ob_drop_scale(ka, 0, DP, DP, B * nh * Sq * Sq, stream)) return 1;
    Pv = g_ws.pd_b;
  }
  if (ob_softmax_causal_bwd_f32(P, DP, B * nh, Sq, stream)) return 1;
  if (gemm(0, 0, Sq, hd, Sq, scale, DP, Sq, nh * Sq * Sq, Sq * Sq, qkv + H,
           3 * H, Sq * 3 * H, hd, 0.f, DQKV, 3 * H, Sq * 3 * H, hd, B, nh,
           nullptr, nullptr, 0, 1, stream))
    return 1;
  if (gemm(1, 0, Sq, hd, Sq, scale, DP, Sq, nh * Sq * Sq, Sq * Sq, qkv, 3 * H,
           Sq * 3 * H, hd, 0.f, DQKV + H, 3 * H, Sq * 3 * H, hd, B, nh,
           nullptr, nullptr, 0, 1, stream))
    return 1;
  if (gemm(1, 0, Sq, hd, Sq, 1.f, Pv, Sq, nh * Sq * Sq, Sq * Sq, DATT, H,
           Sq * H, hd, 0.f, DQKV + 2 * H, 3 * H, Sq * 3 * H, hd, B, nh,
           nullptr, nullptr, 0, 1, stream))
    return 1;
  if (ob_colsum_f32(DQKV, g + bp.b_qkv, BS, 3 * H, stream)) return 1;
  if (gemm(1, 0, H, 3 * H, BS, 1.f, ln1, H, 0, 0, DQKV, 3 * H, 0, 0, 1.f,
           g + bp.w_qkv, 3 * H, 0, 0, 1, 1, nullptr, nullptr, 1,
           pick_splitk(H, 3 * H, BS), stream))
    return 1;
  if (gemm_dx_splitk(1, BS, H, 3 * H, 1.f, DQKV, 3 * H, p + bp.w_qkv, 3 * H,
                     DLN, H, stream))
    return 1;
  if (ob_layernorm_bwd_f32(x, p + bp.ln1_w, st + l->o_mean1, st + l->o_rstd1,
                           DLN, din, g + bp.ln1_w, g + bp.ln1_b, BS, H, 1,
                           stream))
    return 1;
  return 0;
}

static int final_backward(ob_layer* l, int slot, const float* dout, float* din,
                          void* stream) {
  const int64_t Sq = l->d.seq_len, H = l->d.n_embd, V = l->d.vocab_size;
  const int64_t B = l->B, BS = B * Sq;
  float* st = l->stash + (int64_t)slot * l->slot_stride;
  const float* p = l->params;
  float* g = l->grads;
  float* x = st + l->o_x;
  float* lnf = st + l->o_ln1;
  float* logits = st + l->o_logits;
  int64_t* labs = l->ids + (int64_t)slot * (int64_t)l->d.max_batch * Sq;

  if (ob_ce_bwd_f32(logits, labs, st + l->o_lse, (const float*)dout, B, Sq, V,
                    stream))
    return 1;
  if (gemm(1, 0, V, H, BS, 1.f, logits, V, 0, 0, lnf, H, 0, 0, 1.f, g + 2 * H,
           H, 0, 0, 1, 1, nullptr, nullptr, 1, 1, stream))
    return 1;
  if (gemm_dx_splitk(0, BS, H, V, 1.f, logits, V, p + 2 * H, H, g_ws.bsh1, H,
                     stream))
    return 1;
  if (ob_layernorm_bwd_f32(x, p + 0, st + l->o_mean1, st + l->o_rstd1,
                           g_ws.bsh1, din, g + 0, g + H, BS, H, 0, stream))
    return 1;
  return 0;
}

extern "C" int ob_layer_backward(ob_layer_t l, int32_t slot, const void* dout,
                                 void* din, void* stream) {
  if (!l) return ob_fail("backward: null layer");
  if (!l->params || !l->grads) return ob_fail("backward: buffers not bound");
  if (slot < 0 || slot >= l->d.n_slots) return ob_fail("backward: bad slot");
  switch (l->d.kind) {
    case OB_KIND_EMBED: {
      const int64_t Sq = l->d.seq_len, H = l->d.n_embd, V = l->d.vocab_size;
      int64_t* ids = l->ids + (int64_t)slot * (int64_t)l->d.max_batch * Sq;
      if (l->slot_drop[slot])
        return OB_PROF(OB_PF_ELEM, stream,
                       ob_embed_bwd_drop(
                           drop_key(l, slot, OB_DROP_EMBD, l->p_embd),
                           l->d.dtype == 1, ids, dout, l->grads,
                           l->grads + V * H, l->B, Sq, H, stream));
      if (l->d.dtype == 1)
        return OB_PROF(OB_PF_ELEM, stream,
                       ob_embed_bwd_bf16(ids, dout, l->grads,
                                         l->grads + V * H, l->B, Sq, H,
                                         stream));
      return OB_PROF(OB_PF_ELEM, stream,
                     ob_embed_bwd_f32(ids, (const float*)dout, l->grads,
                                      l->grads + V * H, l->B, Sq, H,
                                      stream));
    }
    case OB_KIND_BLOCK:
      if (!dout || !din) return ob_fail("block backward: dout/din required");
      if (l->d.dtype == 1)
        return block_backward_bf16(l, slot, (const __bf16*)dout, (__bf16*)din,
                                   stream);
      return block_backward(l, slot, (const float*)dout, (float*)din, stream);
    case OB_KIND_FINAL:
      if (!din) return ob_fail("final backward: din required");
      if (l->d.dtype == 1)
        return final_backward_bf16(l, slot, (const float*)dout, (__bf16*)din,
                                   stream);
      return final_backward(l, slot, (const float*)dout, (float*)din, stream);
  }
  return ob_fail("backward: bad kind");
}
```

Baseline: 739,300 tokens/s.

## Autotune hipBLASLt algorithms per GEMM shape and reuse tuned choices in plans

Adds an on-device autotuner that benchmarks the top hipBLASLt heuristic candidates for each layer GEMM shape on random data. It rejects candidates whose results drift from the top-1 reference and caches the fastest algorithm index in a table. Plan building then uses the tuned algorithm instead of the first heuristic result. Layer GEMM calls are restructured to take explicit shape descriptors so the tuned shapes can be enumerated ahead of time. The cost is extra one-time tuning work, plus the risk that a candidate that wins in isolation does worse inside the real overlapped schedule.

```diff
diff --git a/include/oobleck_stage.h b/include/oobleck_stage.h
--- a/include/oobleck_stage.h
+++ b/include/oobleck_stage.h
@@ -157,6 +157,16 @@
                        int64_t n1, int64_t n2, int out_kind, int splitk,
                        float beta, int aligned16, int env_mask,
                        const char* force, int32_t* out);
+
+int ob_layer_lt_shapes(const ob_layer_desc* desc, int64_t* out, int cap);
+int ob_gemm_lt_tune(const int64_t* shape);
+int ob_gemm_lt_choice(const int64_t* shape, double* out, char* top1_name,
+                      char* chosen_name, int name_cap);
+int ob_gemm_lt_candidates(const int64_t* shape, int32_t* index, int32_t* pos,
+                          double* us, int cap);
+int64_t ob_gemm_lt_table_size(void);
+int64_t ob_gemm_lt_untuned_uses(void);
+int ob_gemm_lt_plan_index(const int64_t* shape, void* stream);
 
 int ob_flash_fwd_nt_bf16(const void* qkv, void* O, void* lse, int64_t B,
                          int64_t Sq, int64_t H, int64_t nh, float scale,
diff --git a/oobleck_amd/_ext.py b/oobleck_amd/_ext.py
--- a/oobleck_amd/_ext.py
+++ b/oobleck_amd/_ext.py
@@ -129,6 +129,21 @@
     lib.ob_gemm_bf16_route.argtypes = [i32, i32, i64, i64, i64, i64, i64, i32,
                                        i32, f32, i32, i32, ctypes.c_char_p,
                                        ctypes.POINTER(ctypes.c_int32)]
+    lib.ob_gemm_lt_bias_res.argtypes = [i32, i32, i64, i64, i64, f32, vp, i64,
+                                        vp, i64, vp, i64, i32, vp, vp, vp]
+    shape = ctypes.POINTER(i64)
+    lib.ob_layer_lt_shapes.argtypes = [ctypes.POINTER(ObLayerDesc), shape, i32]
+    lib.ob_gemm_lt_tune.argtypes = [shape]
+    lib.ob_gemm_lt_choice.argtypes = [shape, ctypes.POINTER(ctypes.c_double),
+                                      ctypes.c_char_p, ctypes.c_char_p, i32]
+    lib.ob_gemm_lt_candidates.argtypes = [shape, ctypes.POINTER(i32),
+                                          ctypes.POINTER(i32),
+                                          ctypes.POINTER(ctypes.c_double), i32]
+    lib.ob_gemm_lt_table_size.argtypes = []
+    lib.ob_gemm_lt_table_size.restype = i64
+    lib.ob_gemm_lt_untuned_uses.argtypes = []
+    lib.ob_gemm_lt_untuned_uses.restype = i64
+    lib.ob_gemm_lt_plan_index.argtypes = [shape, vp]
     lib.ob_profile_enable.argtypes = [i32]
     lib.ob_profile_enable.restype = None
     lib.ob_profile_reset.argtypes = []
@@ -178,6 +193,52 @@
     return _LIB
 
 
+LT_SHAPE_FIELDS = 13
+LT_SHAPE_NAMES = ("tA", "tB", "M", "N", "K", "lda", "ldb", "ldc", "c_f32",
+                  "beta1", "bias", "cin", "ab_f32")
+
+
+def lt_shape(tA, tB, M, N, K, lda, ldb, ldc, c_f32=0, beta1=0, bias=0, cin=0,
+             ab_f32=0):
+    return (ctypes.c_int64 * LT_SHAPE_FIELDS)(tA, tB, M, N, K, lda, ldb, ldc,
+                                              c_f32, beta1, bias, cin, ab_f32)
+
+
+def layer_lt_shapes(desc: ObLayerDesc) -> list[tuple]:
+    lib = get_ext()
+    n = lib.ob_layer_lt_shapes(ctypes.byref(desc), None, 0)
+    if n < 0:
+        raise RuntimeError("ob_layer_lt_shapes failed")
+    buf = (ctypes.c_int64 * (LT_SHAPE_FIELDS * max(n, 1)))()
+    lib.ob_layer_lt_shapes(ctypes.byref(desc), buf, n)
+    return [tuple(buf[i * LT_SHAPE_FIELDS:(i + 1) * LT_SHAPE_FIELDS])
+            for i in range(n)]
+
+
+def lt_choice(shape) -> dict | None:
+    out = (ctypes.c_double * 10)()
+    top1 = ctypes.create_string_buffer(512)
+    chosen = ctypes.create_string_buffer(512)
+    check(get_ext().ob_gemm_lt_choice(lt_shape(*shape), out, top1, chosen, 512),
+          "gemm_lt_choice")
+    if not out[0]:
+        return None
+    return {"index": int(out[1]), "tuned": bool(out[2]),
+            "top1_index": int(out[3]), "us_top1": out[4], "us_chosen": out[5],
+            "tried": int(out[6]), "dropped": int(out[7]), "wall_ms": out[8],
+            "spread_top1": out[9],
+            "top1_kernel": top1.value.decode(),
+            "chosen_kernel": chosen.value.decode()}
+
+
+def lt_candidates(shape, cap: int = 128) -> list[dict]:
+    idx, pos = (ctypes.c_int32 * cap)(), (ctypes.c_int32 * cap)()
+    us = (ctypes.c_double * cap)()
+    n = get_ext().ob_gemm_lt_candidates(lt_shape(*shape), idx, pos, us, cap)
+    return [{"index": idx[i], "pos": pos[i], "us": us[i]}
+            for i in range(max(0, min(n, cap)))]
+
+
 def check(rc: int, what: str = "") -> None:
     if rc != 0:
         err = get_ext().ob_last_error().decode()
diff --git a/oobleck_amd/csrc/ob_blaslt.hip b/oobleck_amd/csrc/ob_blaslt.hip
--- a/oobleck_amd/csrc/ob_blaslt.hip
+++ b/oobleck_amd/csrc/ob_blaslt.hip
@@ -1,23 +1,45 @@
 #include "ob_internal.h"
 
+#include <hipblaslt/hipblaslt-ext.hpp>
 #include <hipblaslt/hipblaslt.h>
 
+#include <algorithm>
+#include <atomic>
+#include <chrono>
 #include <cstdlib>
+#include <cstring>
 #include <map>
+#include <mutex>
+#include <set>
+#include <string>
 #include <tuple>
+#include <vector>
 
 namespace {
 
-struct LtPlan {
+constexpr size_t kLtWs = 64u << 20;
+
+struct Key {
+  ob_lt_shape s;
+  auto tie() const {
+    return std::tie(s.tA, s.tB, s.M, s.N, s.K, s.lda, s.ldb, s.ldc, s.c_f32,
+                    s.beta1, s.bias, s.cin, s.ab_f32);
+  }
+  bool operator<(const Key& o) const { return tie() < o.tie(); }
+};
+
+struct LtProblem {
   hipblasLtMatmulDesc_t desc = nullptr;
   hipblasLtMatrixLayout_t la = nullptr, lb = nullptr, lc = nullptr;
+};
+
+struct LtPlan {
+  LtProblem p;
   hipblasLtMatmulAlgo_t algo{};
+  int index = -1;
   bool ok = false;
+  bool untuned = false;
 };
-
-constexpr size_t kLtWs = 64u << 20;
-using Key = std::tuple<int, int, int64_t, int64_t, int64_t, int64_t, int,
-                       int, int, int>;
 
 struct LtCtx {
   hipblasLtHandle_t h = nullptr;
@@ -25,6 +47,30 @@
   std::map<Key, LtPlan> plans;
 };
 std::map<void*, LtCtx> g_lt_by_stream;
+
+struct LtChoice {
+  int index = -1;
+  int top1_index = -1;
+  bool tuned = false;
+  double us_top1 = 0, us_chosen = 0;
+  int tried = 0, dropped = 0;
+  double wall_ms = 0;
+  double spread_top1 = 0;
+  std::string top1_name, chosen_name;
+  struct Timed {
+    int index, pos;
+    double us;
+  };
+  std::vector<Timed> timed;
+};
+std::mutex g_tab_mu;
+std::map<Key, LtChoice> g_tab;
+std::atomic<int64_t> g_untuned_uses{0};
+
+bool lt_tune_on() {
+  static const bool on = ob_env_flag("OB_LT_TUNE", true);
+  return on;
+}
 
 LtCtx* lt_ctx(void* stream) {
   auto it = g_lt_by_stream.find(stream);
@@ -35,6 +81,417 @@
   return &g_lt_by_stream.emplace(stream, ctx).first->second;
 }
 
+void lt_problem_create(const ob_lt_shape& k, const void* bias, LtProblem* p) {
+  const hipblasOperation_t opA = k.tB ? HIPBLAS_OP_T : HIPBLAS_OP_N;
+  const hipblasOperation_t opB = k.tA ? HIPBLAS_OP_T : HIPBLAS_OP_N;
+  const int64_t a_rows = k.tB ? k.K : k.N, a_cols = k.tB ? k.N : k.K;
+  const int64_t b_rows = k.tA ? k.M : k.K, b_cols = k.tA ? k.K : k.M;
+  hipblasLtMatmulDescCreate(&p->desc, HIPBLAS_COMPUTE_32F, HIP_R_32F);
+  hipblasLtMatmulDescSetAttribute(p->desc, HIPBLASLT_MATMUL_DESC_TRANSA, &opA,
+                                  sizeof(opA));
+  hipblasLtMatmulDescSetAttribute(p->desc, HIPBLASLT_MATMUL_DESC_TRANSB, &opB,
+                                  sizeof(opB));
+  if (k.bias) {
+    const hipblasLtEpilogue_t ep = HIPBLASLT_EPILOGUE_BIAS;
+    hipblasLtMatmulDescSetAttribute(p->desc, HIPBLASLT_MATMUL_DESC_EPILOGUE,
+                                    &ep, sizeof(ep));
+    const int32_t bt = HIP_R_32F;
+    hipblasLtMatmulDescSetAttribute(
+        p->desc, HIPBLASLT_MATMUL_DESC_BIAS_DATA_TYPE, &bt, sizeof(bt));
+    hipblasLtMatmulDescSetAttribute(
+        p->desc, HIPBLASLT_MATMUL_DESC_BIAS_POINTER, &bias, sizeof(bias));
+  }
+  const hipDataType abt = k.ab_f32 ? HIP_R_32F : HIP_R_16BF;
+  hipblasLtMatrixLayoutCreate(&p->la, abt, a_rows, a_cols, k.ldb);
+  hipblasLtMatrixLayoutCreate(&p->lb, abt, b_rows, b_cols, k.lda);
+  hipblasLtMatrixLayoutCreate(&p->lc, k.c_f32 ? HIP_R_32F : HIP_R_16BF, k.N,
+                              k.M, k.ldc);
+}
+
+void lt_problem_destroy(LtProblem* p) {
+  if (p->la) hipblasLtMatrixLayoutDestroy(p->la);
+  if (p->lb) hipblasLtMatrixLayoutDestroy(p->lb);
+  if (p->lc) hipblasLtMatrixLayoutDestroy(p->lc);
+  if (p->desc) hipblasLtMatmulDescDestroy(p->desc);
+  *p = LtProblem();
+}
+
+int lt_heuristic(hipblasLtHandle_t h, const LtProblem& p, int n,
+                 hipblasLtMatmulHeuristicResult_t* res) {
+  hipblasLtMatmulPreference_t pref;
+  hipblasLtMatmulPreferenceCreate(&pref);
+  const uint64_t ws = kLtWs;
+  hipblasLtMatmulPreferenceSetAttribute(
+      pref, HIPBLASLT_MATMUL_PREF_MAX_WORKSPACE_BYTES, &ws, sizeof(ws));
+  int nres = 0;
+  const hipblasStatus_t st = hipblasLtMatmulAlgoGetHeuristic(
+      h, p.desc, p.la, p.lb, p.lc, p.lc, pref, n, res, &nres);
+  hipblasLtMatmulPreferenceDestroy(pref);
+  return st == HIPBLAS_STATUS_SUCCESS ? nres : 0;
+}
+
+bool lt_algo_from_index(hipblasLtHandle_t h, const LtProblem& p,
+                        const ob_lt_shape& k, int index,
+                        hipblasLtMatmulAlgo_t* algo) {
+  std::vector<int> idx{index};
+  std::vector<hipblasLtMatmulHeuristicResult_t> r;
+  if (hipblaslt_ext::getAlgosFromIndex(h, idx, r) != HIPBLAS_STATUS_SUCCESS ||
+      r.empty())
+    return false;
+  const float alpha = 1.f, beta = k.beta1 ? 1.f : 0.f;
+  size_t need = 0;
+  if (hipblaslt_ext::matmulIsAlgoSupported(h, p.desc, &alpha, p.la, p.lb,
+                                           &beta, p.lc, p.lc, r[0].algo,
+                                           need) != HIPBLAS_STATUS_SUCCESS ||
+      need > kLtWs)
+    return false;
+  *algo = r[0].algo;
+  return true;
+}
+
+LtPlan lt_plan_build(LtCtx* ctx, const Key& key, const void* bias) {
+  LtPlan p;
+  lt_problem_create(key.s, bias, &p.p);
+  int index = -1;
+  {
+    std::lock_guard<std::mutex> lk(g_tab_mu);
+    auto it = g_tab.find(key);
+    if (it == g_tab.end())
+      p.untuned = lt_tune_on();
+    else if (it->second.tuned)
+      index = it->second.index;
+  }
+  if (index >= 0 && lt_algo_from_index(ctx->h, p.p, key.s, index, &p.algo)) {
+    p.index = index;
+    p.ok = true;
+    return p;
+  }
+  hipblasLtMatmulHeuristicResult_t res[1];
+  if (lt_heuristic(ctx->h, p.p, 1, res) > 0 &&
+      res[0].state == HIPBLAS_STATUS_SUCCESS) {
+    p.algo = res[0].algo;
+    p.index = hipblaslt_ext::getIndexFromAlgo(p.algo);
+    p.ok = true;
+  }
+  return p;
+}
+
+
+__global__ void k_lt_fill(void* p, int64_t n, int f32, uint32_t seed) {
+  for (int64_t i = blockIdx.x * (int64_t)blockDim.x + threadIdx.x; i < n;
+       i += (int64_t)gridDim.x * blockDim.x) {
+    uint32_t h = (uint32_t)i * 2654435761u + (uint32_t)(i >> 32) + seed;
+    h ^= h >> 16, h *= 0x7feb352du, h ^= h >> 15, h *= 0x846ca68bu;
+    h ^= h >> 16;
+    const float v = (float)(h >> 16) * (1.f / 32768.f) - 1.f;
+    if (f32) ((float*)p)[i] = v;
+    else ((__bf16*)p)[i] = (__bf16)v;
+  }
+}
+
+__global__ void k_lt_diff(const void* x, const void* ref, int64_t n, int f32,
+                          double* acc) {
+  double d2 = 0, r2 = 0;
+  for (int64_t i = blockIdx.x * (int64_t)blockDim.x + threadIdx.x; i < n;
+       i += (int64_t)gridDim.x * blockDim.x) {
+    const float a = f32 ? ((const float*)x)[i] : (float)((const __bf16*)x)[i];
+    const float b =
+        f32 ? ((const float*)ref)[i] : (float)((const __bf16*)ref)[i];
+    d2 += (double)(a - b) * (a - b);
+    r2 += (double)b * b;
+  }
+  __shared__ double sd[256], sr[256];
+  sd[threadIdx.x] = d2, sr[threadIdx.x] = r2;
+  __syncthreads();
+  for (int s = 128; s > 0; s >>= 1) {
+    if ((int)threadIdx.x < s) {
+      sd[threadIdx.x] += sd[threadIdx.x + s];
+      sr[threadIdx.x] += sr[threadIdx.x + s];
+    }
+    __syncthreads();
+  }
+  if (threadIdx.x == 0) {
+    atomicAdd(&acc[0], sd[0]);
+    atomicAdd(&acc[1], sr[0]);
+  }
+}
+
+double median_of(std::vector<float> v) {
+  std::sort(v.begin(), v.end());
+  return v[v.size() / 2];
+}
+
+struct TuneScratch {
+  hipStream_t stream = nullptr;
+  hipblasLtHandle_t h = nullptr;
+  void *ws = nullptr, *A = nullptr, *B = nullptr, *C = nullptr, *Cref = nullptr,
+       *Cin = nullptr, *bias = nullptr;
+  double* acc = nullptr;
+  hipEvent_t e0 = nullptr, e1 = nullptr;
+  LtProblem p;
+  ~TuneScratch() {
+    lt_problem_destroy(&p);
+    for (void* q : {ws, A, B, C, Cref, Cin, bias, (void*)acc})
+      if (q) (void)hipFree(q);
+    if (e0) (void)hipEventDestroy(e0);
+    if (e1) (void)hipEventDestroy(e1);
+    if (h) hipblasLtDestroy(h);
+    if (stream) (void)hipStreamDestroy(stream);
+  }
+};
+
+struct Cand {
+  hipblasLtMatmulAlgo_t algo;
+  int pos = 0;
+  int reps = 1;
+  float warm_us = 0.f;
+  std::vector<float> us;
+};
+
+bool lt_tune_run(const ob_lt_shape& k, LtChoice* out) {
+  const int n_env = ob_env_int("OB_LT_TUNE_N", 8);
+  const int n_max = n_env < 1 ? 1 : n_env > 128 ? 128 : n_env;
+  constexpr int kRounds = 5;
+  TuneScratch t;
+#define LT_TRY(x) \
+  if ((x) != hipSuccess) return false
+  LT_TRY(hipStreamCreateWithFlags(&t.stream, hipStreamNonBlocking));
+  if (hipblasLtCreate(&t.h) != HIPBLAS_STATUS_SUCCESS) return false;
+  LT_TRY(hipEventCreate(&t.e0));
+  LT_TRY(hipEventCreate(&t.e1));
+  const size_t es_ab = k.ab_f32 ? 4 : 2, es_c = k.c_f32 ? 4 : 2;
+  const int64_t nA = (k.tA ? k.K : k.M) * k.lda;
+  const int64_t nB = (k.tB ? k.N : k.K) * k.ldb;
+  const int64_t nC = k.M * k.ldc;
+  LT_TRY(hipMalloc(&t.ws, kLtWs));
+  LT_TRY(hipMalloc(&t.A, nA * es_ab));
+  LT_TRY(hipMalloc(&t.B, nB * es_ab));
+  LT_TRY(hipMalloc(&t.C, nC * es_c));
+  LT_TRY(hipMalloc(&t.Cref, nC * es_c));
+  LT_TRY(hipMalloc((void**)&t.acc, 2 * sizeof(double)));
+  if (k.cin) LT_TRY(hipMalloc(&t.Cin, nC * es_c));
+  if (k.bias) LT_TRY(hipMalloc(&t.bias, k.N * sizeof(float)));
+  auto fill = [&](void* p, int64_t n, int f32, uint32_t seed) {
+    const int64_t blocks = std::min<int64_t>((n + 255) / 256, 4096);
+    k_lt_fill<<<(unsigned)blocks, 256, 0, t.stream>>>(p, n, f32, seed);
+  };
+  fill(t.A, nA, k.ab_f32, 1u);
+  fill(t.B, nB, k.ab_f32, 2u);
+  if (t.Cin) fill(t.Cin, nC, k.c_f32, 3u);
+  if (t.bias) fill(t.bias, k.N, 1, 4u);
+  LT_TRY(hipGetLastError());
+  lt_problem_create(k, t.bias, &t.p);
+
+  std::vector<hipblasLtMatmulHeuristicResult_t> res(n_max);
+  res.resize(std::max(0, lt_heuristic(t.h, t.p, n_max, res.data())));
+  if (res.empty() || res[0].state != HIPBLAS_STATUS_SUCCESS) return false;
+  out->top1_index = hipblaslt_ext::getIndexFromAlgo(res[0].algo);
+  out->top1_name = hipblaslt_ext::getKernelNameFromAlgo(t.h, res[0].algo);
+
+  const float alpha = 1.f, beta = k.beta1 ? 1.f : 0.f;
+  if (ob_env_flag("OB_LT_TUNE_ALL", false)) {
+    std::vector<hipblasLtMatmulHeuristicResult_t> every;
+    const hipDataType abt = k.ab_f32 ? HIP_R_32F : HIP_R_16BF;
+    const hipDataType ct = k.c_f32 ? HIP_R_32F : HIP_R_16BF;
+    if (hipblaslt_ext::getAllAlgos(
+            t.h, hipblaslt_ext::GemmType::HIPBLASLT_GEMM,
+            k.tB ? HIPBLAS_OP_T : HIPBLAS_OP_N,
+            k.tA ? HIPBLAS_OP_T : HIPBLAS_OP_N, abt, abt, ct, ct,
+            HIPBLAS_COMPUTE_32F, every) == HIPBLAS_STATUS_SUCCESS) {
+      std::set<int> seen;
+      for (auto& r : res) seen.insert(hipblaslt_ext::getIndexFromAlgo(r.algo));
+      for (auto& r : every) {
+        size_t need = 0;
+        if (!seen.insert(hipblaslt_ext::getIndexFromAlgo(r.algo)).second)
+          continue;
+        if (hipblaslt_ext::matmulIsAlgoSupported(
+                t.h, t.p.desc, &alpha, t.p.la, t.p.lb, &beta, t.p.lc, t.p.lc,
+                r.algo, need) != HIPBLAS_STATUS_SUCCESS ||
+            need > kLtWs)
+          continue;
+        r.state = HIPBLAS_STATUS_SUCCESS;
+        res.push_back(r);
+      }
+    }
+  }
+  const int nres = (int)res.size();
+  auto run = [&](hipblasLtMatmulAlgo_t& algo, void* dst) {
+    return hipblasLtMatmul(t.h, t.p.desc, &alpha, t.B, t.p.la, t.A, t.p.lb,
+                           &beta, t.Cin ? t.Cin : dst, t.p.lc, dst, t.p.lc,
+                           &algo, t.ws, kLtWs, t.stream);
+  };
+  const double bound = k.c_f32 ? 1e-3 : 1.0 / 256;
+  std::vector<Cand> cands;
+  for (int i = 0; i < nres; i++) {
+    if (res[i].state != HIPBLAS_STATUS_SUCCESS) {
+      out->dropped++;
+      continue;
+    }
+    void* dst = i == 0 ? t.Cref : t.C;
+    LT_TRY(hipMemsetAsync(dst, 0, nC * es_c, t.stream));
+    const hipblasStatus_t st = run(res[i].algo, dst);
+    if (i == 0 && st != HIPBLAS_STATUS_SUCCESS) return false;
+    if (st != HIPBLAS_STATUS_SUCCESS) {
+      LT_TRY(hipStreamSynchronize(t.stream));
+      out->dropped++;
+      continue;
+    }
+    if (i > 0) {
+      LT_TRY(hipMemsetAsync(t.acc, 0, 2 * sizeof(double), t.stream));
+      const int64_t blocks = std::min<int64_t>((nC + 255) / 256, 4096);
+      k_lt_diff<<<(unsigned)blocks, 256, 0, t.stream>>>(t.C, t.Cref, nC,
+                                                        k.c_f32, t.acc);
+      double acc[2] = {0, 0};
+      LT_TRY(hipMemcpyAsync(acc, t.acc, sizeof(acc), hipMemcpyDeviceToHost,
+                            t.stream));
+      LT_TRY(hipStreamSynchronize(t.stream));
+      if (!(acc[0] <= bound * bound * acc[1])) {
+        out->dropped++;
+        continue;
+      }
+    } else {
+      LT_TRY(hipStreamSynchronize(t.stream));
+    }
+    Cand c;
+    c.algo = res[i].algo;
+    c.pos = i;
+    cands.push_back(c);
+  }
+  out->tried = nres;
+  enum { V_OK = 0, V_DROP = 1, V_HIP = 2 };
+  auto visit = [&](Cand& c, int reps, float* us) {
+    if (hipEventRecord(t.e0, t.stream) != hipSuccess) return (int)V_HIP;
+    bool lib_ok = true;
+    for (int r = 0; r < reps && lib_ok; r++)
+      lib_ok = run(c.algo, t.C) == HIPBLAS_STATUS_SUCCESS;
+    float ms = 0.f;
+    if (hipEventRecord(t.e1, t.stream) != hipSuccess ||
+        hipEventSynchronize(t.e1) != hipSuccess ||
+        hipEventElapsedTime(&ms, t.e0, t.e1) != hipSuccess)
+      return (int)V_HIP;
+    if (!lib_ok) return (int)V_DROP;
+    *us = ms * 1000.f / reps;
+    return (int)V_OK;
+  };
+  auto drop = [&](size_t i) {
+    if (i == 0) return false;
+    cands.erase(cands.begin() + i);
+    out->dropped++;
+    return true;
+  };
+  auto reps_for = [](float us) {
+    return std::max(1, std::min(4096, (int)(1250.f / std::max(us, 0.25f)) + 1));
+  };
+  LT_TRY(hipMemsetAsync(t.C, 0, nC * es_c, t.stream));
+  for (size_t i = 0; i < cands.size();) {
+    Cand& c = cands[i];
+    float us = 0.f;
+    int v = visit(c, 1, &us);
+    if (v == V_OK) v = visit(c, 8, &us);
+    if (v == V_HIP || (v == V_DROP && !drop(i))) return false;
+    if (v == V_DROP) continue;
+    c.warm_us = us;
+    c.reps = reps_for(us);
+    i++;
+  }
+  if ((int)cands.size() > n_max) {
+    std::stable_sort(cands.begin() + 1, cands.end(),
+                     [](const Cand& a, const Cand& b) {
+                       return a.warm_us < b.warm_us;
+                     });
+    cands.resize(n_max);
+  }
+  for (int r = 0; r < kRounds; r++)
+    for (size_t i = 0; i < cands.size();) {
+      Cand& c = cands[i];
+      float us = 0.f;
+      int v = V_OK;
+      for (int attempt = 0; attempt < 4; attempt++) {
+        v = visit(c, c.reps, &us);
+        if (v != V_OK || us * c.reps >= 1000.f || c.reps >= 4096) break;
+        c.reps = std::max(c.reps + 1, reps_for(us));
+      }
+      if (v == V_HIP || (v == V_DROP && !drop(i))) return false;
+      if (v == V_DROP) continue;
+      c.us.push_back(us);
+      i++;
+    }
+  LT_TRY(hipStreamSynchronize(t.stream));
+#undef LT_TRY
+  const double med0 = median_of(cands[0].us);
+  const double spread0 =
+      *std::max_element(cands[0].us.begin(), cands[0].us.end()) -
+      *std::min_element(cands[0].us.begin(), cands[0].us.end());
+  size_t best = 0;
+  double best_med = med0;
+  out->timed.push_back(
+      {hipblaslt_ext::getIndexFromAlgo(cands[0].algo), 0, med0});
+  for (size_t i = 1; i < cands.size(); i++) {
+    const double m = median_of(cands[i].us);
+    out->timed.push_back(
+        {hipblaslt_ext::getIndexFromAlgo(cands[i].algo), cands[i].pos, m});
+    if (m < best_med) best_med = m, best = i;
+  }
+  out->spread_top1 = spread0;
+  const double min0 =
+      *std::min_element(cands[0].us.begin(), cands[0].us.end());
+  if (!(best_med < med0 - spread0) ||
+      !(*std::max_element(cands[best].us.begin(), cands[best].us.end()) <
+        min0))
+    best = 0, best_med = med0;
+  out->us_top1 = med0;
+  out->us_chosen = best_med;
+  out->index = hipblaslt_ext::getIndexFromAlgo(cands[best].algo);
+  out->chosen_name = hipblaslt_ext::getKernelNameFromAlgo(t.h, cands[best].algo);
+  out->tuned = true;
+  return true;
+}
+
+Key key_from_i64(const int64_t* v) {
+  Key key;
+  ob_lt_shape& s = key.s;
+  s.tA = v[0] != 0, s.tB = v[1] != 0, s.M = v[2], s.N = v[3], s.K = v[4];
+  s.lda = v[5], s.ldb = v[6], s.ldc = v[7], s.c_f32 = v[8] != 0;
+  s.beta1 = v[9] != 0, s.bias = v[10] != 0, s.cin = v[11] != 0;
+  s.ab_f32 = v[12] != 0;
+  return key;
+}
+
+}
+
+int ob_lt_tune_shape(const ob_lt_shape& s) {
+  if (!lt_tune_on()) return 0;
+  if (s.M <= 0 || s.N <= 0 || s.K <= 0 || s.ldc < s.N ||
+      s.lda < (s.tA ? s.M : s.K) || s.ldb < (s.tB ? s.K : s.N))
+    return ob_fail("lt_tune: bad shape");
+  const Key key{s};
+  {
+    std::lock_guard<std::mutex> lk(g_tab_mu);
+    if (g_tab.count(key)) return 0;
+  }
+  OB_HIP(hipDeviceSynchronize());
+  const auto t0 = std::chrono::steady_clock::now();
+  LtChoice c;
+  if (!lt_tune_run(s, &c)) {
+    c.tuned = false;
+    c.index = c.top1_index;
+    (void)hipGetLastError();
+  }
+  (void)hipDeviceSynchronize();
+  c.wall_ms = std::chrono::duration<double, std::milli>(
+                  std::chrono::steady_clock::now() - t0)
+                  .count();
+  {
+    std::lock_guard<std::mutex> lk(g_tab_mu);
+    g_tab.emplace(key, c);
+  }
+  for (auto& sc : g_lt_by_stream) {
+    auto it = sc.second.plans.find(key);
+    if (it == sc.second.plans.end()) continue;
+    lt_problem_destroy(&it->second.p);
+    sc.second.plans.erase(it);
+  }
+  return 0;
 }
 
 static int lt_matmul(int tA, int tB, int64_t M, int64_t N, int64_t K,
@@ -45,61 +502,20 @@
   if (!Cin) Cin = C;
   LtCtx* ctx = lt_ctx(stream);
   if (!ctx) return ob_fail("hipblasLt per-stream context init failed");
-  const Key key{tA,     tB,           M,
-                N,      K,            ldc,
-                c_f32,  beta != 0.f,  bias != nullptr,
-                ab_f32};
+  const Key key{ob_lt_shape_of(tA, tB, M, N, K, lda, ldb, ldc, c_f32, beta,
+                               bias != nullptr, Cin != C, ab_f32)};
   auto it = ctx->plans.find(key);
-  if (it == ctx->plans.end()) {
-    LtPlan p;
-    const hipblasOperation_t opA = tB ? HIPBLAS_OP_T : HIPBLAS_OP_N;
-    const hipblasOperation_t opB = tA ? HIPBLAS_OP_T : HIPBLAS_OP_N;
-    const int64_t a_rows = tB ? K : N, a_cols = tB ? N : K;
-    const int64_t b_rows = tA ? M : K, b_cols = tA ? K : M;
-    hipblasLtMatmulDescCreate(&p.desc, HIPBLAS_COMPUTE_32F, HIP_R_32F);
-    hipblasLtMatmulDescSetAttribute(p.desc, HIPBLASLT_MATMUL_DESC_TRANSA,
-                                    &opA, sizeof(opA));
-    hipblasLtMatmulDescSetAttribute(p.desc, HIPBLASLT_MATMUL_DESC_TRANSB,
-                                    &opB, sizeof(opB));
-    if (bias) {
-      const hipblasLtEpilogue_t ep = HIPBLASLT_EPILOGUE_BIAS;
-      hipblasLtMatmulDescSetAttribute(p.desc, HIPBLASLT_MATMUL_DESC_EPILOGUE,
-                                      &ep, sizeof(ep));
-      const int32_t bt = HIP_R_32F;
-      hipblasLtMatmulDescSetAttribute(
-          p.desc, HIPBLASLT_MATMUL_DESC_BIAS_DATA_TYPE, &bt, sizeof(bt));
-      hipblasLtMatmulDescSetAttribute(
-          p.desc, HIPBLASLT_MATMUL_DESC_BIAS_POINTER, &bias, sizeof(bias));
-    }
-    const hipDataType abt = ab_f32 ? HIP_R_32F : HIP_R_16BF;
-    hipblasLtMatrixLayoutCreate(&p.la, abt, a_rows, a_cols, ldb);
-    hipblasLtMatrixLayoutCreate(&p.lb, abt, b_rows, b_cols, lda);
-    hipblasLtMatrixLayoutCreate(&p.lc, c_f32 ? HIP_R_32F : HIP_R_16BF, N, M,
-                                ldc);
-    hipblasLtMatmulPreference_t pref;
-    hipblasLtMatmulPreferenceCreate(&pref);
-    const uint64_t ws = kLtWs;
-    hipblasLtMatmulPreferenceSetAttribute(
-        pref, HIPBLASLT_MATMUL_PREF_MAX_WORKSPACE_BYTES, &ws, sizeof(ws));
-    hipblasLtMatmulHeuristicResult_t res[1];
-    int nres = 0;
-    hipblasLtMatmulAlgoGetHeuristic(ctx->h, p.desc, p.la, p.lb, p.lc, p.lc,
-                                    pref, 1, res, &nres);
-    hipblasLtMatmulPreferenceDestroy(pref);
-    if (nres > 0 && res[0].state == HIPBLAS_STATUS_SUCCESS) {
-      p.algo = res[0].algo;
-      p.ok = true;
-    }
-    it = ctx->plans.emplace(key, p).first;
-  }
+  if (it == ctx->plans.end())
+    it = ctx->plans.emplace(key, lt_plan_build(ctx, key, bias)).first;
   const LtPlan& p = it->second;
   if (!p.ok) return -1;
+  if (p.untuned) g_untuned_uses.fetch_add(1, std::memory_order_relaxed);
   if (bias)
     hipblasLtMatmulDescSetAttribute(
-        p.desc, HIPBLASLT_MATMUL_DESC_BIAS_POINTER, &bias, sizeof(bias));
+        p.p.desc, HIPBLASLT_MATMUL_DESC_BIAS_POINTER, &bias, sizeof(bias));
   const hipblasStatus_t st = hipblasLtMatmul(
-      ctx->h, p.desc, &alpha, B, p.la, A, p.lb, &beta, Cin, p.lc, C, p.lc,
-      &p.algo, ctx->ws, kLtWs, reinterpret_cast<hipStream_t>(stream));
+      ctx->h, p.p.desc, &alpha, B, p.p.la, A, p.p.lb, &beta, Cin, p.p.lc, C,
+      p.p.lc, &p.algo, ctx->ws, kLtWs, reinterpret_cast<hipStream_t>(stream));
   if (st != HIPBLAS_STATUS_SUCCESS)
     return ob_fail("hipblasLtMatmul failed (%d)", (int)st);
   return 0;
@@ -140,3 +556,65 @@
   return lt_matmul(tA, tB, M, N, K, alpha, A, lda, B, ldb, beta, C, ldc, 1,
                    nullptr, 1, stream);
 }
+
+
+extern "C" int ob_gemm_lt_tune(const int64_t* shape) {
+  if (!shape) return ob_fail("gemm_lt_tune: null shape");
+  return ob_lt_tune_shape(key_from_i64(shape).s);
+}
+
+extern "C" int ob_gemm_lt_choice(const int64_t* shape, double* out,
+                                 char* top1_name, char* chosen_name,
+                                 int name_cap) {
+  if (!shape || !out) return ob_fail("gemm_lt_choice: null argument");
+  const Key key = key_from_i64(shape);
+  std::lock_guard<std::mutex> lk(g_tab_mu);
+  auto it = g_tab.find(key);
+  for (int i = 0; i < 10; i++) out[i] = 0;
+  if (top1_name && name_cap > 0) top1_name[0] = 0;
+  if (chosen_name && name_cap > 0) chosen_name[0] = 0;
+  if (it == g_tab.end()) return 0;
+  const LtChoice& c = it->second;
+  out[0] = 1, out[1] = c.index, out[2] = c.tuned, out[3] = c.top1_index;
+  out[4] = c.us_top1, out[5] = c.us_chosen, out[6] = c.tried;
+  out[7] = c.dropped, out[8] = c.wall_ms, out[9] = c.spread_top1;
+  if (top1_name && name_cap > 0)
+    snprintf(top1_name, name_cap, "%s", c.top1_name.c_str());
+  if (chosen_name && name_cap > 0)
+    snprintf(chosen_name, name_cap, "%s", c.chosen_name.c_str());
+  return 0;
+}
+
+extern "C" int ob_gemm_lt_candidates(const int64_t* shape, int32_t* index,
+                                     int32_t* pos, double* us, int cap) {
+  if (!shape || (cap > 0 && (!index || !pos || !us))) return -1;
+  std::lock_guard<std::mutex> lk(g_tab_mu);
+  auto it = g_tab.find(key_from_i64(shape));
+  if (it == g_tab.end()) return 0;
+  auto v = it->second.timed;
+  std::stable_sort(v.begin(), v.end(),
+                   [](const LtChoice::Timed& a, const LtChoice::Timed& b) {
+                     return a.us < b.us;
+                   });
+  for (int i = 0; i < (int)v.size() && i < cap; i++)
+    index[i] = v[i].index, pos[i] = v[i].pos, us[i] = v[i].us;
+  return (int)v.size();
+}
+
+extern "C" int64_t ob_gemm_lt_table_size(void) {
+  std::lock_guard<std::mutex> lk(g_tab_mu);
+  return (int64_t)g_tab.size();
+}
+
+extern "C" int64_t ob_gemm_lt_untuned_uses(void) {
+  return g_untuned_uses.load(std::memory_order_relaxed);
+}
+
+extern "C" int ob_gemm_lt_plan_index(const int64_t* shape, void* stream) {
+  if (!shape) return -1;
+  auto sc = g_lt_by_stream.find(stream);
+  if (sc == g_lt_by_stream.end()) return -1;
+  auto it = sc->second.plans.find(key_from_i64(shape));
+  return it == sc->second.plans.end() || !it->second.ok ? -1
+                                                        : it->second.index;
+}
diff --git a/oobleck_amd/csrc/ob_internal.h b/oobleck_amd/csrc/ob_internal.h
--- a/oobleck_amd/csrc/ob_internal.h
+++ b/oobleck_amd/csrc/ob_internal.h
@@ -193,6 +193,38 @@
                               int64_t lda, const void* B, int64_t ldb,
                               float beta, void* C, int64_t ldc,
                               void* stream);
+struct ob_lt_shape {
+  int tA = 0, tB = 0;
+  int64_t M = 0, N = 0, K = 0, lda = 0, ldb = 0, ldc = 0;
+  int c_f32 = 0;
+  int beta1 = 0;
+  int bias = 0;
+  int cin = 0;
+  int ab_f32 = 0;
+};
+#define OB_LT_SHAPE_FIELDS 13
+inline ob_lt_shape ob_lt_shape_of(int tA, int tB, int64_t M, int64_t N,
+                                  int64_t K, int64_t lda, int64_t ldb,
+                                  int64_t ldc, int c_f32, float beta,
+                                  bool bias, bool cin, int ab_f32) {
+  ob_lt_shape s;
+  s.tA = tA != 0, s.tB = tB != 0, s.M = M, s.N = N, s.K = K;
+  s.lda = lda, s.ldb = ldb, s.ldc = ldc, s.c_f32 = c_f32 != 0;
+  s.beta1 = beta != 0.f, s.bias = bias, s.cin = cin, s.ab_f32 = ab_f32 != 0;
+  return s;
+}
+inline ob_lt_shape ob_lt_linear(int64_t M, int64_t K, int64_t N, bool bias,
+                                bool res) {
+  return ob_lt_shape_of(0, 1, M, N, K, K, K, N, 0, res ? 1.f : 0.f, bias, res,
+                        0);
+}
+inline ob_lt_shape ob_lt_dw(int64_t actw, int64_t dyw, int64_t BS,
+                            int64_t lda) {
+  return ob_lt_shape_of(1, 0, actw, dyw, BS, lda, dyw, dyw, 1, 1.f, false,
+                        false, 0);
+}
+int ob_lt_tune_shape(const ob_lt_shape& s);
+
 struct ob_bf16_gemm {
   const void* A = nullptr;
   const void* B = nullptr;
diff --git a/oobleck_amd/csrc/ob_layer.hip b/oobleck_amd/csrc/ob_layer.hip
--- a/oobleck_amd/csrc/ob_layer.hip
+++ b/oobleck_amd/csrc/ob_layer.hip
@@ -1,8 +1,10 @@
+#include "ob_gemm_route.h"
 #include "ob_internal.h"
 #include "ob_philox.h"
 
 #include <cmath>
 #include <cstring>
+#include <initializer_list>
 #include <vector>
 
 static inline hipStream_t S(void* s) { return reinterpret_cast<hipStream_t>(s); }
@@ -222,6 +224,10 @@
   }
   return -1;
 }
+
+static void ob_layer_lt_list(const ob_layer_desc* d, bool resid_drop,
+                             std::vector<ob_lt_shape>* out);
+static int64_t v_pad_of(int64_t V) { return (V + 255) / 256 * 256; }
 
 static int layer_create(const ob_layer_desc* d, const ob_dropout_desc* drop,
                         ob_layer_t* out) {
@@ -302,7 +308,7 @@
       return ob_fail("create: ids hipMalloc failed");
     }
   }
-  l->v_pad = (V + 255) / 256 * 256;
+  l->v_pad = v_pad_of(V);
   if (d->dtype == 1) {
     int64_t o2 = 0;
     if (d->kind == OB_KIND_BLOCK) {
@@ -362,6 +368,13 @@
   if (l->p_resid > 0.f) {
     if (ws_ensure(&g_ws.dm1, &g_ws.sz_dm1, BSH)) return 1;
     if (ws_ensure(&g_ws.dm2, &g_ws.sz_dm2, BSH)) return 1;
+  }
+  static const bool no_lt = ob_env_flag("OB_NO_BLASLT", false);
+  if (!no_lt) {
+    std::vector<ob_lt_shape> shapes;
+    ob_layer_lt_list(d, l->p_resid > 0.f, &shapes);
+    for (const ob_lt_shape& s : shapes)
+      if (ob_lt_tune_shape(s)) return 1;
   }
   *out = l;
   return 0;
@@ -605,13 +618,91 @@
 }
 
 
-static int linear_bf(const void* in, int64_t M, int64_t K, const void* W,
-                     int64_t N, const float* bias, const void* res, void* out,
+enum {
+  LG_QKV = 0, LG_AP, LG_FC, LG_MP,
+  LG_DX_MP, LG_DX_FC, LG_DX_AP, LG_DX_QKV,
+  LG_DW_MP, LG_DW_FC, LG_DW_AP, LG_DW_QKV,
+  LG_BLOCK_N
+};
+enum { LG_LM = 0, LG_DLNOUT, LG_DW_LM, LG_FINAL_N };
+
+static void block_gemms(int64_t H, int64_t BS, bool res, ob_lt_shape* g) {
+  g[LG_QKV] = ob_lt_linear(BS, H, 3 * H, true, false);
+  g[LG_AP] = ob_lt_linear(BS, H, H, true, res);
+  g[LG_FC] = ob_lt_linear(BS, H, 4 * H, true, false);
+  g[LG_MP] = ob_lt_linear(BS, 4 * H, H, true, res);
+  g[LG_DX_MP] = ob_lt_linear(BS, H, 4 * H, false, false);
+  g[LG_DX_FC] = ob_lt_linear(BS, 4 * H, H, false, false);
+  g[LG_DX_AP] = ob_lt_linear(BS, H, H, false, false);
+  g[LG_DX_QKV] = ob_lt_linear(BS, 3 * H, H, false, false);
+  g[LG_DW_MP] = ob_lt_dw(4 * H, H, BS, 4 * H);
+  g[LG_DW_FC] = ob_lt_dw(H, 4 * H, BS, H);
+  g[LG_DW_AP] = ob_lt_dw(H, H, BS, H);
+  g[LG_DW_QKV] = ob_lt_dw(H, 3 * H, BS, H);
+}
+
+static void final_gemms(int64_t H, int64_t V, int64_t v_pad, int64_t BS,
+                        ob_lt_shape* g) {
+  g[LG_LM] = ob_lt_linear(BS, H, v_pad, false, false);
+  g[LG_DLNOUT] = ob_lt_linear(BS, v_pad, H, false, false);
+  g[LG_DW_LM] = ob_lt_dw(V, H, BS, v_pad);
+}
+
+static bool lt_routed(const ob_lt_shape& s) {
+  if (s.tA) return true;
+  const ob_gemm_env env = {false, false, false, nullptr};
+  return ob_gemm_bf16_pick(0, 1, s.M, s.N, s.K, 1, 1, BF_OUT_BF16, 1, 0.f,
+                           true, env)
+      .try_lt_first;
+}
+
+static void ob_layer_lt_list(const ob_layer_desc* d, bool resid_drop,
+                             std::vector<ob_lt_shape>* out) {
+  if (d->dtype != 1) return;
+  const int64_t H = d->n_embd, V = d->vocab_size;
+  const int64_t BS = (int64_t)d->max_batch * d->seq_len;
+  ob_lt_shape g[LG_BLOCK_N];
+  int n = 0;
+  if (d->kind == OB_KIND_BLOCK) {
+    block_gemms(H, BS, true, g);
+    n = LG_BLOCK_N;
+  } else if (d->kind == OB_KIND_FINAL) {
+    final_gemms(H, V, v_pad_of(V), BS, g);
+    n = LG_FINAL_N;
+  }
+  for (int i = 0; i < n; i++)
+    if (lt_routed(g[i])) out->push_back(g[i]);
+  if (d->kind == OB_KIND_BLOCK && resid_drop) {
+    block_gemms(H, BS, false, g);
+    for (int i : {LG_AP, LG_MP})
+      if (lt_routed(g[i])) out->push_back(g[i]);
+  }
+}
+
+extern "C" int ob_layer_lt_shapes(const ob_layer_desc* d, int64_t* out,
+                                  int cap) {
+  if (!d || (!out && cap > 0)) return -1;
+  std::vector<ob_lt_shape> v;
+  ob_layer_lt_list(d, false, &v);
+  for (int i = 0; i < (int)v.size() && i < cap; i++) {
+    const ob_lt_shape& s = v[i];
+    int64_t* o = out + (int64_t)i * OB_LT_SHAPE_FIELDS;
+    o[0] = s.tA, o[1] = s.tB, o[2] = s.M, o[3] = s.N, o[4] = s.K;
+    o[5] = s.lda, o[6] = s.ldb, o[7] = s.ldc, o[8] = s.c_f32, o[9] = s.beta1;
+    o[10] = s.bias, o[11] = s.cin, o[12] = s.ab_f32;
+  }
+  return (int)v.size();
+}
+
+static int linear_bf(const ob_lt_shape& s, const void* in, const void* W,
+                     const float* bias, const void* res, void* out,
                      void* stream) {
+  if ((bias != nullptr) != (s.bias != 0) || (res != nullptr) != (s.cin != 0))
+    return ob_fail("linear_bf: operands do not match the listed shape");
   ob_bf16_gemm g;
   g.A = in, g.B = W, g.C = out, g.bias = bias, g.residual = res;
-  g.M = M, g.N = N, g.K = K, g.lda = K, g.ldb = K, g.ldc = N;
-  g.stream = stream;
+  g.M = s.M, g.N = s.N, g.K = s.K, g.lda = s.lda, g.ldb = s.ldb;
+  g.ldc = s.ldc, g.stream = stream;
   return ob_gemm_bf16_run(g);
 }
 
@@ -624,13 +715,14 @@
   return g;
 }
 
-static int dw_bf16_ws(const __bf16* act, int64_t actw, const __bf16* dY,
-                      int64_t dyw, int64_t BS, float* gout, int64_t ldc,
-                      float* w1, float* w2, void* stream) {
+static int dw_bf16_ws(const ob_lt_shape& s, const __bf16* act,
+                      const __bf16* dY, float* gout, float* w1, float* w2,
+                      void* stream) {
+  const int64_t actw = s.M, dyw = s.N, BS = s.K, ldc = s.ldc;
   static const bool no_lt = ob_env_flag("OB_NO_BLASLT", false);
-  if (!no_lt && ldc == dyw) {
-    const int r = ob_gemm_lt(1, 0, actw, dyw, BS, 1.f, act, actw, dY, dyw,
-                             1.f, gout, ldc, 1, stream);
+  if (!no_lt) {
+    const int r = ob_gemm_lt(s.tA, s.tB, s.M, s.N, s.K, 1.f, act, s.lda, dY,
+                             s.ldb, 1.f, gout, s.ldc, s.c_f32, stream);
     if (r >= 0) return r;
   }
   ob_bf16_gemm g;
@@ -660,6 +752,8 @@
   const BlockParams bp = block_params(H);
   const bool dA = l->slot_drop[slot] && l->p_attn > 0.f;
   const bool dR = l->slot_drop[slot] && l->p_resid > 0.f;
+  ob_lt_shape lg[LG_BLOCK_N];
+  block_gemms(H, BS, !dR, lg);
 
   __bf16* x = (__bf16*)(st + l->o_x);
   __bf16* ln1 = (__bf16*)(st + l->o_ln1);
@@ -670,7 +764,7 @@
     return 1;
   __bf16* qkv = (__bf16*)(st + l->o_qkv);
   if (OB_PROF(OB_PF_GEMM_FWD, stream,
-              linear_bf(ln1, BS, H, sh + l->sh_qkv_t, 3 * H, p + bp.b_qkv,
+              linear_bf(lg[LG_QKV], ln1, sh + l->sh_qkv_t, p + bp.b_qkv,
                         nullptr, qkv, stream)))
     return 1;
   __bf16* am = (__bf16*)(st + l->o_attnm);
@@ -725,7 +819,7 @@
   }
   __bf16* hmid = (__bf16*)(st + l->o_hmid);
   if (OB_PROF(OB_PF_GEMM_FWD, stream,
-              linear_bf(am, BS, H, sh + l->sh_ap_t, H, p + bp.b_attnproj,
+              linear_bf(lg[LG_AP], am, sh + l->sh_ap_t, p + bp.b_attnproj,
                         dR ? nullptr : x, hmid, stream)))
     return 1;
   if (dR &&
@@ -741,7 +835,7 @@
     return 1;
   __bf16* u = (__bf16*)(st + l->o_u);
   if (OB_PROF(OB_PF_FC_FWD, stream,
-              linear_bf(ln2, BS, H, sh + l->sh_fc_t, 4 * H, p + bp.b_fc,
+              linear_bf(lg[LG_FC], ln2, sh + l->sh_fc_t, p + bp.b_fc,
                         nullptr, u, stream)))
     return 1;
   __bf16* gact = (__bf16*)(st + l->o_g);
@@ -749,7 +843,7 @@
               ob_gelu_fwd_bf16(u, gact, BS * 4 * H, stream)))
     return 1;
   if (OB_PROF(OB_PF_GEMM_FWD, stream,
-              linear_bf(gact, BS, 4 * H, sh + l->sh_mp_t, H,
+              linear_bf(lg[LG_MP], gact, sh + l->sh_mp_t,
                         p + bp.b_mlpproj, dR ? nullptr : hmid, out, stream)))
     return 1;
   if (dR &&
@@ -768,6 +862,8 @@
   float* st = l->stash + (int64_t)slot * l->slot_stride;
   const float* p = l->params;
   if (!labels) return ob_fail("final_forward_bf16: labels required");
+  ob_lt_shape lg[LG_FINAL_N];
+  final_gemms(H, V, l->v_pad, BS, lg);
 
   __bf16* x = (__bf16*)(st + l->o_x);
   int64_t* labs = l->ids + (int64_t)slot * (int64_t)l->d.max_batch * Sq;
@@ -781,7 +877,7 @@
     return 1;
   __bf16* logits = (__bf16*)(st + l->o_logits);
   if (OB_PROF(OB_PF_GEMM_FWD, stream,
-              linear_bf(lnf, BS, H, l->shadows + l->sh_lm, l->v_pad, nullptr,
+              linear_bf(lg[LG_LM], lnf, l->shadows + l->sh_lm, nullptr,
                         nullptr, logits, stream)))
     return 1;
   OB_HIP(hipMemsetAsync(out, 0, sizeof(float), S(stream)));
@@ -821,6 +917,8 @@
   __bf16* DP = (__bf16*)g_ws.dp;
   const bool dA = l->slot_drop[slot] && l->p_attn > 0.f;
   const bool dR = l->slot_drop[slot] && l->p_resid > 0.f;
+  ob_lt_shape lg[LG_BLOCK_N];
+  block_gemms(H, BS, !dR, lg);
 
   void* const side = (void*)g_side.stream;
   OB_SIDE_FENCE(S(stream), g_side.stream);
@@ -836,11 +934,11 @@
     OB_SIDE_FENCE(S(stream), g_side.stream);
   }
   if (OB_PROF(OB_PF_GEMM_DX, stream,
-              linear_bf(dmlp, BS, H, sh + l->sh_mp, 4 * H, nullptr, nullptr,
+              linear_bf(lg[LG_DX_MP], dmlp, sh + l->sh_mp, nullptr, nullptr,
                         DY4, stream)))
     return 1;
   if (OB_PROF(OB_PF_GEMM_DW, side,
-              dw_bf16_ws(gact, 4 * H, dmlp, H, BS, g + bp.w_mlpproj, H,
+              dw_bf16_ws(lg[LG_DW_MP], gact, dmlp, g + bp.w_mlpproj,
                          g_ws.s1, g_ws.s2, side)))
     return 1;
   if (OB_PROF(OB_PF_ELEM, stream,
@@ -849,11 +947,11 @@
     return 1;
   OB_SIDE_FENCE(S(stream), g_side.stream);
   if (OB_PROF(OB_PF_GEMM_DW, side,
-              dw_bf16_ws(ln2, H, DY4, 4 * H, BS, g + bp.w_fc, 4 * H, g_ws.s1,
+              dw_bf16_ws(lg[LG_DW_FC], ln2, DY4, g + bp.w_fc, g_ws.s1,
                          g_ws.s2, side)))
     return 1;
   if (OB_PROF(OB_PF_GEMM_DX, stream,
-              linear_bf(DY4, BS, 4 * H, sh + l->sh_fc, H, nullptr, nullptr,
+              linear_bf(lg[LG_DX_FC], DY4, sh + l->sh_fc, nullptr, nullptr,
                         DLN, stream)))
     return 1;
   if (OB_PROF(OB_PF_LN, stream,
@@ -875,11 +973,11 @@
   }
   OB_SIDE_FENCE(S(stream), g_side.stream);
   if (OB_PROF(OB_PF_GEMM_DX, stream,
-              linear_bf(dap, BS, H, sh + l->sh_ap, H, nullptr, nullptr, DATT,
+              linear_bf(lg[LG_DX_AP], dap, sh + l->sh_ap, nullptr, nullptr, DATT,
                         stream)))
     return 1;
   if (OB_PROF(OB_PF_GEMM_DW, side,
-              dw_bf16_ws(am, H, dap, H, BS, g + bp.w_attnproj, H, g_ws.s1,
+              dw_bf16_ws(lg[LG_DW_AP], am, dap, g + bp.w_attnproj, g_ws.s1,
                          g_ws.s2, side)))
     return 1;
   hipEvent_t ev_din_done = side_evt();
@@ -967,11 +1065,11 @@
               ob_colsum_bf16(DQKV, g + bp.b_qkv, BS, 3 * H, side)))
     return 1;
   if (OB_PROF(OB_PF_GEMM_DW, side,
-              dw_bf16_ws(ln1, H, DQKV, 3 * H, BS, g + bp.w_qkv, 3 * H,
+              dw_bf16_ws(lg[LG_DW_QKV], ln1, DQKV, g + bp.w_qkv,
                          g_ws.s1, g_ws.s2, side)))
     return 1;
   if (OB_PROF(OB_PF_GEMM_DX, stream,
-              linear_bf(DQKV, BS, 3 * H, sh + l->sh_qkv, H, nullptr, nullptr,
+              linear_bf(lg[LG_DX_QKV], DQKV, sh + l->sh_qkv, nullptr, nullptr,
                         DLN, stream)))
     return 1;
   OB_HIP(hipStreamWaitEvent(S(stream), ev_din_done, 0));
@@ -996,6 +1094,9 @@
   __bf16* logits = (__bf16*)(st + l->o_logits);
   int64_t* labs = l->ids + (int64_t)slot * (int64_t)l->d.max_batch * Sq;
   __bf16* DLN = (__bf16*)g_ws.bsh1;
+  ob_lt_shape lg[LG_FINAL_N];
+  final_gemms(H, V, l->v_pad, BS, lg);
+  const ob_lt_shape& dwlm = lg[LG_DW_LM];
 
   if (OB_PROF(OB_PF_CE, stream,
               ob_ce_bwd_bf16(logits, labs, st + l->o_lse, dout, B, Sq, V,
@@ -1008,8 +1109,9 @@
     int r = -1;
     if (!no_lt)
       r = OB_PROF(OB_PF_GEMM_DW, side,
-                  ob_gemm_lt(1, 0, V, H, BS, 1.f, logits, l->v_pad, lnf, H,
-                             1.f, g + 2 * H, H, 1, side));
+                  ob_gemm_lt(dwlm.tA, dwlm.tB, dwlm.M, dwlm.N, dwlm.K, 1.f,
+                             logits, dwlm.lda, lnf, dwlm.ldb, 1.f, g + 2 * H,
+                             dwlm.ldc, dwlm.c_f32, side));
     if (r > 0) return 1;
     if (r < 0) {
       __bf16* DLT = (__bf16*)g_ws.s1;
@@ -1025,7 +1127,7 @@
     }
   }
   if (OB_PROF(OB_PF_GEMM_DX, stream,
-              linear_bf(logits, BS, l->v_pad, l->shadows + l->sh_lm_t, H,
+              linear_bf(lg[LG_DLNOUT], logits, l->shadows + l->sh_lm_t,
                         nullptr, nullptr, DLN, stream)))
     return 1;
   if (OB_PROF(OB_PF_LN, stream,
```

Result: faster. 757,500 tokens/s, median of 6 (+2.5%).
